# jesusbriales/dvo_slam

Measured on AMD Instinct MI355X. Metric: frame-pairs/s (640x480, 4-level GN align), higher is better.
Workload: dtype f32

## Files before the change

dvo_slam_amd/capi.py:

```python
from __future__ import annotations

import ctypes as C
import dataclasses
import os

import numpy as np

from . import _build

MAX_LEVELS = 8
TERMINATION = {0: "IterationsExceeded", 1: "IncrementTooSmall", 2: "LogLikelihoodDecreased", 3: "TooFewConstraints",
               -1: "Unset"}

EXPORTS = [
    "dvo_amd_abi_version", "dvo_amd_build_id", "dvo_amd_status_string", "dvo_amd_last_error", "dvo_amd_device_count",
    "dvo_amd_default_config", "dvo_amd_context_create", "dvo_amd_context_destroy", "dvo_amd_configure",
    "dvo_amd_get_config", "dvo_amd_pyramid_create", "dvo_amd_pyramid_create_from_device", "dvo_amd_pyramid_retain",
    "dvo_amd_pyramid_release", "dvo_amd_pyramid_levels", "dvo_amd_pyramid_timestamp", "dvo_amd_pyramid_level_info",
    "dvo_amd_pyramid_download_plane", "dvo_amd_pyramid_select", "dvo_amd_match", "dvo_amd_match_batch",
    "dvo_amd_residuals", "dvo_amd_error_image", "dvo_amd_kernel_timing", "dvo_amd_se3_exp", "dvo_amd_se3_log",
    "dvo_amd_solve6", "dvo_amd_bench_residual_pass", "dvo_amd_match_many",
    "dvo_amd_debug_finalize_stamps", "dvo_amd_comm_unique_id", "dvo_amd_comm_create", "dvo_amd_comm_destroy",
    "dvo_amd_match_sharded", "dvo_amd_match_banded", "dvo_amd_context_device", "dvo_amd_debug_combine_bands", "dvo_amd_debug_wire_layout", "dvo_amd_debug_take_wire", "dvo_amd_pyramid_create_raw",
    "dvo_amd_default_validator_stages", "dvo_amd_proposals_for_candidates", "dvo_amd_validate_proposals",
    "dvo_amd_track_frame", "dvo_amd_png_info", "dvo_amd_png_read_bgr8", "dvo_amd_png_read_gray16",
    "dvo_amd_format_trajectory_line", "dvo_amd_debug_tick_log", "dvo_amd_debug_iteration", "dvo_amd_match_selection", "dvo_amd_bench_residual_pass_pairs",
    "dvo_amd_exchange_create", "dvo_amd_exchange_attach", "dvo_amd_exchange_destroy",
    "dvo_amd_match_submit", "dvo_amd_match_wait", "dvo_amd_match_poll", "dvo_amd_debug_next_seq",
    "dvo_amd_set_reciprocal_mode", "dvo_amd_get_reciprocal_mode", "dvo_amd_debug_rcp", "dvo_amd_debug_block_trace",
    "dvo_amd_debug_ll_overflow", "dvo_amd_debug_marker", "dvo_amd_debug_rcp_form", "dvo_amd_debug_weights", "dvo_amd_debug_hw_queue",
    "dvo_amd_debug_level_geometry", "dvo_amd_point_cloud", "dvo_amd_map_cloud", "dvo_amd_voxel_downsample", "dvo_amd_write_pcd",
    "dvo_amd_debug_map_timing", "dvo_amd_default_graph_options", "dvo_amd_optimize_graph", "dvo_amd_graph_marginals", "dvo_amd_debug_graph_timing",
    "dvo_amd_debug_graph_system", "dvo_amd_debug_graph_system_sparse", "dvo_amd_debug_graph_symbolic",
    "dvo_amd_debug_graph_sparse_timing", "dvo_amd_optimize_graphs_batch", "dvo_amd_debug_graph_batch_records",
    "dvo_amd_debug_tick_layout",
    "dvo_amd_map_create", "dvo_amd_map_destroy", "dvo_amd_map_insert", "dvo_amd_map_set_poses", "dvo_amd_map_remove",
    "dvo_amd_map_stats", "dvo_amd_map_extract", "dvo_amd_map_render", "dvo_amd_map_render_pyramid", "dvo_amd_debug_keyframe_map_timing", "dvo_amd_debug_map_merge",
    "dvo_amd_default_covisibility_options", "dvo_amd_covisibility", "dvo_amd_find_constraint_candidates",
    "dvo_amd_debug_covisibility_ms",
    "dvo_amd_remap_create", "dvo_amd_remap_create_undistort", "dvo_amd_remap_retain", "dvo_amd_remap_release", "dvo_amd_remap_info",
    "dvo_amd_remap_download", "dvo_amd_pyramid_create_raw_remapped", "dvo_amd_debug_ingest_timing",
    "dvo_amd_default_registration", "dvo_amd_pyramid_create_raw_registered",
    "dvo_amd_pyramid_create_raw_batch", "dvo_amd_debug_batch_build_stats",
    "dvo_amd_mask_create", "dvo_amd_mask_create_levels", "dvo_amd_mask_retain", "dvo_amd_mask_release", "dvo_amd_mask_info",
    "dvo_amd_mask_download", "dvo_amd_pyramid_select_masked", "dvo_amd_match_masked", "dvo_amd_match_many_masked",
    "dvo_amd_default_budget_options", "dvo_amd_mask_create_budget",
    "dvo_amd_default_mask_warp_options", "dvo_amd_mask_combine", "dvo_amd_mask_morph", "dvo_amd_mask_warp", "dvo_amd_mask_warp_many",
    "dvo_amd_debug_mask_ops_timing",
    "dvo_amd_default_residual_mask_options", "dvo_amd_mask_from_residuals", "dvo_amd_mask_from_residuals_many",
    "dvo_amd_default_fuse_options", "dvo_amd_pyramid_fuse_depth", "dvo_amd_pyramid_fuse_depth_many", "dvo_amd_debug_fuse_timing",
    "dvo_amd_default_place_options", "dvo_amd_default_place_query_options", "dvo_amd_place_index_create", "dvo_amd_place_index_destroy",
    "dvo_amd_place_index_add", "dvo_amd_place_index_info", "dvo_amd_place_index_download", "dvo_amd_place_scores", "dvo_amd_place_query",
    "dvo_amd_place_query_frames", "dvo_amd_debug_place_timing",
    "dvo_amd_debug_residuals_masked", "dvo_amd_debug_iteration_masked", "dvo_amd_debug_weights_masked",
    "dvo_amd_default_normal_options", "dvo_amd_pyramid_normals", "dvo_amd_mask_from_normals", "dvo_amd_point_cloud_normals",
    "dvo_amd_write_pcd_normals", "dvo_amd_debug_normals_timing",
    "dvo_amd_default_depth_filter_options", "dvo_amd_pyramid_filter_depth", "dvo_amd_pyramid_filter_depth_many",
    "dvo_amd_debug_depth_filter_timing",
    "dvo_amd_default_component_options", "dvo_amd_mask_filter_components", "dvo_amd_mask_filter_components_many",
    "dvo_amd_mask_components", "dvo_amd_debug_components_timing",
    "dvo_amd_default_pose_score_options", "dvo_amd_score_poses", "dvo_amd_score_poses_many", "dvo_amd_rank_poses", "dvo_amd_pose_grid",
    "dvo_amd_default_exposure_options", "dvo_amd_estimate_exposure", "dvo_amd_estimate_exposure_many",
    "dvo_amd_pyramid_adjust_intensity", "dvo_amd_pyramid_adjust_intensity_many", "dvo_amd_debug_exposure_timing",
    "dvo_amd_default_warp_options", "dvo_amd_warp_inverse", "dvo_amd_warp_inverse_many", "dvo_amd_pyramid_warp_inverse",
    "dvo_amd_pyramid_warp_inverse_many", "dvo_amd_warp_forward", "dvo_amd_warp_forward_many", "dvo_amd_pyramid_warp_forward",
    "dvo_amd_pyramid_warp_forward_many", "dvo_amd_debug_warp_timing",
    "dvo_amd_default_volume_options", "dvo_amd_default_volume_raycast_options", "dvo_amd_volume_create", "dvo_amd_volume_destroy",
    "dvo_amd_volume_clear", "dvo_amd_volume_options_get", "dvo_amd_volume_integrate", "dvo_amd_volume_insert",
    "dvo_amd_volume_set_poses", "dvo_amd_volume_remove", "dvo_amd_volume_stats", "dvo_amd_volume_download", "dvo_amd_volume_raycast",
    "dvo_amd_volume_raycast_pyramid", "dvo_amd_volume_extract", "dvo_amd_debug_volume_timing",
    "dvo_amd_volume_mesh", "dvo_amd_volume_upload", "dvo_amd_write_ply",
]


class CConfig(C.Structure):
    _fields_ = [("first_level", C.c_int), ("last_level", C.c_int), ("max_iterations_per_level", C.c_int),
                ("precision", C.c_double), ("mu", C.c_double), ("use_initial_estimate", C.c_int),
                ("intensity_derivative_threshold", C.c_float), ("depth_derivative_threshold", C.c_float),
                ("segment_geometry", C.c_int), ("reserved", C.c_int)]


GEOMETRY_THROUGHPUT, GEOMETRY_LATENCY = 0, 1


class CIterationStats(C.Structure):
    _fields_ = [("id", C.c_int), ("valid_constraints", C.c_int), ("tdist_loglik", C.c_double),
                ("tdist_mean", C.c_double * 2), ("tdist_precision", C.c_double * 4), ("prior_loglik", C.c_double),
                ("increment", C.c_double * 6), ("information", C.c_double * 36), ("has_increment", C.c_int),
                ("reserved", C.c_int), ("estimate", C.c_double * 16), ("initial", C.c_double * 16)]


class CLevelStats(C.Structure):
    _fields_ = [("id", C.c_int), ("max_valid_pixels", C.c_int), ("valid_pixels", C.c_int), ("termination", C.c_int),
                ("n_iterations", C.c_int), ("first_iteration", C.c_int)]


class CResult(C.Structure):
    _fields_ = [("transformation", C.c_double * 16), ("information", C.c_double * 36), ("loglik", C.c_double),
                ("is_nan", C.c_int), ("n_levels", C.c_int), ("levels", CLevelStats * MAX_LEVELS),
                ("n_iterations", C.c_int), ("iterations_capacity", C.c_int),
                ("iterations", C.POINTER(CIterationStats)), ("n_ticks", C.c_int), ("n_residual_passes", C.c_int),
                ("alg_bytes", C.c_double), ("alg_bytes_discarded", C.c_double)]


class CFrameCriteria(C.Structure):
    _fields_ = [("odometry_is_nan", C.c_int), ("keyframe_is_nan", C.c_int), ("odometry_translation_norm", C.c_double),
                ("keyframe_translation_norm", C.c_double), ("keyframe_constraint_ratio", C.c_double),
                ("odometry_neg_loglik", C.c_double), ("keyframe_neg_loglik", C.c_double),
                ("odometry_condition_number", C.c_double), ("keyframe_condition_number", C.c_double)]


class CIterationProbe(C.Structure):
    _fields_ = [("valid_constraints", C.c_int), ("reserved", C.c_int), ("scale_sums", C.c_double * 3),
                ("scale", C.c_float * 4), ("precision", C.c_float * 4), ("moments", C.c_double * 87),
                ("information", C.c_double * 36), ("rhs", C.c_double * 6), ("loglik_sum", C.c_double),
                ("loglik", C.c_float), ("reserved_f", C.c_float)]


class CQ7Probe(C.Structure):
# ... 323 lines not shown
    L.dvo_amd_voxel_downsample.argtypes = [vp, C.c_longlong, vp, C.c_float, vp, C.c_longlong, C.POINTER(CCloudStats)]
    L.dvo_amd_write_pcd.argtypes = [C.c_char_p, vp, C.c_longlong, C.c_int, C.c_int]
    L.dvo_amd_debug_map_timing.argtypes = [vp, dp, dp, C.POINTER(C.c_longlong)]
    L.dvo_amd_map_create.argtypes = [vp, C.c_float, C.POINTER(vp)]
    L.dvo_amd_map_destroy.argtypes = [vp]
    L.dvo_amd_map_destroy.restype = None
    L.dvo_amd_map_insert.argtypes = [vp, C.c_int, vp, dp, vp, C.c_int]
    L.dvo_amd_map_set_poses.argtypes = [vp, C.c_int, C.POINTER(C.c_int), dp]
    L.dvo_amd_map_remove.argtypes = [vp, C.c_int, C.POINTER(C.c_int)]
    L.dvo_amd_map_stats.argtypes = [vp, C.POINTER(CCloudStats), C.POINTER(C.c_int)]
    L.dvo_amd_map_extract.argtypes = [vp, C.POINTER(C.c_float), vp, C.c_longlong, C.POINTER(C.c_longlong)]
    L.dvo_amd_map_render.argtypes = [vp, dp, C.POINTER(CView), vp, vp, vp, vp, C.POINTER(CRenderStats)]
    L.dvo_amd_map_render_pyramid.argtypes = [vp, dp, C.POINTER(CView), C.c_int, C.c_double, C.POINTER(vp), C.POINTER(CRenderStats)]
    L.dvo_amd_debug_keyframe_map_timing.argtypes = [vp, dp, dp, C.POINTER(C.c_longlong), C.POINTER(C.c_longlong),
                                                    C.POINTER(C.c_int)]
    L.dvo_amd_debug_map_merge.argtypes = [vp, C.c_longlong, vp, vp, C.c_longlong, vp, vp, vp, vp, C.POINTER(C.c_longlong)]
    L.dvo_amd_default_covisibility_options.argtypes = [C.POINTER(CCovisibilityOptions)]
    L.dvo_amd_default_covisibility_options.restype = None
    L.dvo_amd_covisibility.argtypes = [vp, C.c_int, C.POINTER(CKeyframe), C.POINTER(CCovisibilityOptions), C.c_int,
                                       C.POINTER(C.c_int), C.POINTER(C.c_int), vp]
    L.dvo_amd_find_constraint_candidates.argtypes = [vp, C.c_int, C.POINTER(CKeyframe), C.c_int, C.c_float, C.c_double,
                                                     C.POINTER(CCovisibilityOptions), C.POINTER(C.c_int), dp, C.c_int,
                                                     C.POINTER(C.c_int)]
    L.dvo_amd_debug_covisibility_ms.argtypes = [vp, dp]
    L.dvo_amd_remap_create.argtypes = [C.c_int, C.c_int, C.c_int, fp, fp, C.c_int, C.c_int, C.c_int, C.POINTER(vp)]
    L.dvo_amd_remap_create_undistort.argtypes = [C.c_int, C.c_int, C.c_int, fp, C.c_int, C.c_int, fp, fp, C.POINTER(vp)]
    L.dvo_amd_remap_retain.argtypes = [vp]
    L.dvo_amd_remap_retain.restype = None
    L.dvo_amd_remap_release.argtypes = [vp]
    L.dvo_amd_remap_release.restype = None
    L.dvo_amd_remap_info.argtypes = [vp, ip, ip, ip, ip, ip]
    L.dvo_amd_remap_download.argtypes = [vp, fp, fp]
    L.dvo_amd_pyramid_create_raw_remapped.argtypes = [C.c_int, vp, C.c_int, C.c_int, vp, C.c_int, C.c_float, C.c_int, vp,
                                                      C.c_float, C.c_float, C.c_float, C.c_float, C.c_int, C.c_double,
                                                      C.POINTER(vp)]
    L.dvo_amd_debug_ingest_timing.argtypes = [C.c_int, C.c_int, dp]
    L.dvo_amd_default_registration.argtypes = [C.POINTER(CRegistration)]
    L.dvo_amd_default_registration.restype = None
    L.dvo_amd_pyramid_create_raw_registered.argtypes = [C.c_int, vp, C.c_int, C.c_int, vp, C.c_int, C.c_float, C.c_int,
                                                        C.POINTER(CRegistration), vp, C.c_int, C.c_int, C.c_float, C.c_float,
                                                        C.c_float, C.c_float, C.c_int, C.c_double, C.POINTER(vp),
                                                        C.POINTER(CRegistrationStats)]
    L.dvo_amd_pyramid_create_raw_batch.argtypes = [C.c_int, C.POINTER(CRawBatch), C.POINTER(vp)]
    L.dvo_amd_debug_batch_build_stats.argtypes = [C.c_int, ip, ip, ip]
    L.dvo_amd_mask_create.argtypes = [C.c_int, C.c_int, C.c_int, C.c_int, vp, C.c_int, C.c_int, C.c_int, C.POINTER(vp)]
    L.dvo_amd_mask_create_levels.argtypes = [C.c_int, C.c_int, C.c_int, C.c_int, C.POINTER(vp), ip, C.c_int, C.POINTER(vp)]
    L.dvo_amd_mask_retain.argtypes = [vp]
    L.dvo_amd_mask_retain.restype = None
    L.dvo_amd_mask_release.argtypes = [vp]
    L.dvo_amd_mask_release.restype = None
    L.dvo_amd_mask_info.argtypes = [vp, ip, ip, ip, C.POINTER(C.c_longlong)]
    L.dvo_amd_mask_download.argtypes = [vp, C.c_int, C.POINTER(C.c_ubyte)]
    L.dvo_amd_pyramid_select_masked.argtypes = [vp, C.c_int, C.c_float, C.c_float, vp, C.POINTER(C.c_int), C.POINTER(C.c_ubyte)]
    L.dvo_amd_match_masked.argtypes = [vp, vp, vp, C.c_float, C.c_float, vp, dp, C.POINTER(CResult)]
    L.dvo_amd_match_many_masked.argtypes = [vp, C.c_int, C.POINTER(vp), C.POINTER(vp), C.POINTER(vp), dp, C.POINTER(CResult), C.c_int]
    L.dvo_amd_default_budget_options.argtypes = [C.POINTER(BudgetOptions)]
    L.dvo_amd_default_budget_options.restype = None
    L.dvo_amd_mask_create_budget.argtypes = [vp, C.POINTER(BudgetOptions), C.POINTER(vp)]
    L.dvo_amd_default_mask_warp_options.argtypes = [C.POINTER(MaskWarpOptions)]
    L.dvo_amd_default_mask_warp_options.restype = None
    L.dvo_amd_mask_combine.argtypes = [vp, vp, C.c_int, C.POINTER(vp)]
    L.dvo_amd_mask_morph.argtypes = [vp, C.c_int, ip, C.POINTER(vp)]
    L.dvo_amd_mask_warp.argtypes = [vp, vp, vp, dp, C.POINTER(MaskWarpOptions), C.POINTER(vp), C.POINTER(C.c_longlong)]
    L.dvo_amd_mask_warp_many.argtypes = [C.c_int, C.POINTER(vp), C.POINTER(vp), C.POINTER(vp), dp, C.POINTER(MaskWarpOptions),
                                         C.POINTER(vp), C.POINTER(C.c_longlong)]
    L.dvo_amd_debug_mask_ops_timing.argtypes = [C.c_int, C.c_int, dp]
    L.dvo_amd_default_residual_mask_options.argtypes = [C.POINTER(ResidualMaskOptions)]
    L.dvo_amd_default_residual_mask_options.restype = None
    L.dvo_amd_mask_from_residuals.argtypes = [vp, vp, vp, dp, C.POINTER(ResidualMaskOptions), C.POINTER(vp), C.POINTER(C.c_longlong),
                                              C.POINTER(C.POINTER(C.c_float))]
    L.dvo_amd_mask_from_residuals_many.argtypes = [vp, C.c_int, C.POINTER(vp), C.POINTER(vp), dp, C.POINTER(ResidualMaskOptions),
                                                   C.POINTER(vp), C.POINTER(C.c_longlong)]
    L.dvo_amd_default_pose_score_options.argtypes = [C.POINTER(PoseScoreOptions)]
    L.dvo_amd_default_pose_score_options.restype = None
    L.dvo_amd_score_poses.argtypes = [vp, vp, vp, C.c_int, dp, C.POINTER(PoseScoreOptions), vp]
    L.dvo_amd_score_poses_many.argtypes = [vp, C.c_int, C.POINTER(vp), C.POINTER(vp), ip, dp, C.POINTER(PoseScoreOptions), vp]
    L.dvo_amd_rank_poses.argtypes = [vp, C.c_int, C.c_int, ip, ip]
    L.dvo_amd_pose_grid.argtypes = [C.POINTER(PoseGridOptions), dp, dp, C.c_int, ip]
    L.dvo_amd_default_exposure_options.argtypes = [C.POINTER(ExposureOptions)]
    L.dvo_amd_default_exposure_options.restype = None
    L.dvo_amd_estimate_exposure.argtypes = [vp, vp, vp, dp, vp, C.POINTER(ExposureOptions), C.POINTER(ExposureEstimate)]
    L.dvo_amd_estimate_exposure_many.argtypes = [vp, C.c_int, C.POINTER(vp), C.POINTER(vp), dp, C.POINTER(vp),
                                                 C.POINTER(ExposureOptions), C.POINTER(ExposureEstimate)]
    L.dvo_amd_pyramid_adjust_intensity.argtypes = [vp, C.c_double, C.c_double, C.POINTER(vp)]
    L.dvo_amd_pyramid_adjust_intensity_many.argtypes = [C.c_int, C.POINTER(vp), dp, dp, C.POINTER(vp)]
    L.dvo_amd_debug_exposure_timing.argtypes = [C.c_int, C.c_int, dp]
    L.dvo_amd_default_warp_options.argtypes = [C.POINTER(WarpOptions)]
    L.dvo_amd_default_warp_options.restype = None
    ll, wo, cv = C.POINTER(C.c_longlong), C.POINTER(WarpOptions), C.POINTER(CView)
    L.dvo_amd_warp_inverse.argtypes = [vp, vp, dp, C.c_int, wo, fp, fp, ll]
    L.dvo_amd_warp_inverse_many.argtypes = [C.c_int, C.POINTER(vp), C.POINTER(vp), dp, C.c_int, wo, C.POINTER(vp), C.POINTER(vp), ll]
    L.dvo_amd_pyramid_warp_inverse.argtypes = [vp, vp, dp, wo, C.POINTER(vp), ll]
    L.dvo_amd_pyramid_warp_inverse_many.argtypes = [C.c_int, C.POINTER(vp), C.POINTER(vp), dp, wo, C.POINTER(vp), ll]
    L.dvo_amd_warp_forward.argtypes = [vp, dp, cv, C.c_int, wo, fp, fp, ip, ll]
    L.dvo_amd_warp_forward_many.argtypes = [C.c_int, C.POINTER(vp), dp, cv, C.c_int, wo, C.POINTER(vp), C.POINTER(vp), C.POINTER(vp), ll]
    L.dvo_amd_pyramid_warp_forward.argtypes = [vp, dp, cv, wo, C.POINTER(vp), ll]
    L.dvo_amd_pyramid_warp_forward_many.argtypes = [C.c_int, C.POINTER(vp), dp, cv, wo, C.POINTER(vp), ll]
    L.dvo_amd_debug_warp_timing.argtypes = [C.c_int, C.c_int, ip, ip, dp]
    vo, ro = C.POINTER(VolumeOptions), C.POINTER(VolumeRaycastOptions)
    L.dvo_amd_default_volume_options.argtypes = [vo]
    L.dvo_amd_default_volume_options.restype = None
    L.dvo_amd_default_volume_raycast_options.argtypes = [ro]
    L.dvo_amd_default_volume_raycast_options.restype = None
    L.dvo_amd_volume_create.argtypes = [C.c_int, vo, C.POINTER(vp)]
    L.dvo_amd_volume_destroy.argtypes = [vp]
    L.dvo_amd_volume_destroy.restype = None
# ... 1017 lines not shown
        b.timestamps = None if timestamps is None else (C.c_double * n)(*[float(t) for t in timestamps])
        b.channels, b.image_stride_bytes, b.depth_stride = channels, image_stride_bytes or w * channels, depth_stride or w
        b.depth_scale, b.on_device, b.width, b.height = depth_scale, int(on_device), w, h
        b.fx, b.fy, b.ox, b.oy = [float(k) for k in K]
        b.levels, b.build_selection = levels, int(selection is not None)
        if selection is not None:
            b.intensity_threshold, b.depth_threshold = float(selection[0]), float(selection[1])
        out = (C.c_void_p * n)()
        _check(lib().dvo_amd_pyramid_create_raw_batch(device, C.byref(b), out), "dvo_amd_pyramid_create_raw_batch")
        del keep
        pyramids = []
        for f in range(n):
            self = cls.__new__(cls)
            self._h, self.device, self.registration_stats = C.c_void_p(out[f]), device, None
            pyramids.append(self)
        return pyramids

    def __del__(self):
        h = getattr(self, "_h", None)
        if h:
            lib().dvo_amd_pyramid_release(h)
            self._h = None

    def levels(self) -> int:
        return lib().dvo_amd_pyramid_levels(self._h)

    def timestamp(self) -> float:
        return lib().dvo_amd_pyramid_timestamp(self._h)

    def level_info(self, level: int):
        w, h = C.c_int(), C.c_int()
        k = np.zeros(4, np.float32)
        _check(lib().dvo_amd_pyramid_level_info(self._h, level, C.byref(w), C.byref(h), _fp(k)), "level_info")
        return w.value, h.value, k

    def plane(self, level: int, plane: int) -> np.ndarray:
        w, h, _ = self.level_info(level)
        out = np.empty((h, w), np.float32)
        _check(lib().dvo_amd_pyramid_download_plane(self._h, level, plane, _fp(out)), "download_plane")
        return out

    def select(self, level: int, ti: float = 0.0, td: float = 0.0, mask: "SelectionMask | None" = None):
        w, h, _ = self.level_info(level)
        out = np.empty((h, w), np.uint8)
        cnt = C.c_int()
        if mask is not None:
            _check(lib().dvo_amd_pyramid_select_masked(self._h, level, ti, td, mask._h, C.byref(cnt),
                                                       out.ctypes.data_as(C.POINTER(C.c_ubyte))), "pyramid_select_masked")
            return cnt.value, out
        _check(lib().dvo_amd_pyramid_select(self._h, level, ti, td, C.byref(cnt),
                                            out.ctypes.data_as(C.POINTER(C.c_ubyte))), "pyramid_select")
        return cnt.value, out


    def fuse_depth(self, frames, transformations, options=None, counts: bool = False, observations: bool = False):
        got = RgbdImagePyramid.fuse_depth_many([self], [frames], [transformations], options, counts=counts, observations=observations)
        return tuple(part[0] for part in got) if counts or observations else got[0]

    @staticmethod
    def fuse_depth_many(keyframes, frames_per_keyframe, transformations_per_keyframe, options=None, counts: bool = False,
                        observations: bool = False):
        nk = len(keyframes)
        if not (len(frames_per_keyframe) == len(transformations_per_keyframe) == nk):
            raise ValueError("one list of frames and one list of transformations per keyframe")
        if any(len(f) != len(t) for f, t in zip(frames_per_keyframe, transformations_per_keyframe)):
            raise ValueError("one transformation per frame")
        opt = options if isinstance(options, FuseOptions) else fuse_options(**(options or {}))
        vp = C.c_void_p
        offsets = np.concatenate([[0], np.cumsum([len(f) for f in frames_per_keyframe])]).astype(np.int32)
        total = int(offsets[-1])
        flat = [p for f in frames_per_keyframe for p in f]
        T = np.ascontiguousarray(np.stack([_pose_cm(t) for ts in transformations_per_keyframe for t in ts]) if total
                                 else np.zeros((1, 4, 4)), dtype=np.float64)
        frame_cnt = np.zeros(max(1, total), FUSE_FRAME_DTYPE)
        key_cnt = np.zeros(max(1, nk), FUSE_KEYFRAME_DTYPE)
        planes = []
        for kf in keyframes:
            w, h, _ = kf.level_info(0)
            planes.append(np.zeros((h, w), np.uint8))
        out = (vp * max(1, nk))()
        obs = (vp * max(1, nk))(*[p.ctypes.data for p in planes]) if observations else None
        ll = C.POINTER(C.c_longlong)
        _check(lib().dvo_amd_pyramid_fuse_depth_many(nk, (vp * max(1, nk))(*[p._h for p in keyframes]),
                                                     offsets.ctypes.data_as(C.POINTER(C.c_int)),
                                                     (vp * max(1, total))(*[p._h for p in flat]), T.ctypes.data_as(C.POINTER(C.c_double)),
                                                     C.byref(opt), out, frame_cnt.ctypes.data_as(ll) if counts else None,
                                                     key_cnt.ctypes.data_as(ll) if counts else None, obs),
               "dvo_amd_pyramid_fuse_depth_many")
        made = []
        for j in range(nk):
            p = RgbdImagePyramid.__new__(RgbdImagePyramid)
            p._h, p.device, p.registration_stats = vp(out[j]), keyframes[j].device, None
            made.append(p)
        result = (made,)
        if counts:
            result += ([frame_cnt[offsets[j]:offsets[j + 1]].copy() for j in range(nk)], key_cnt[:nk].copy())
        if observations:
            result += (planes,)
        return result if len(result) > 1 else made


    def warp_inverse(self, fixed: "RgbdImagePyramid", T, level=None, options=None):
        got = warp_inverse_many([fixed], [self], [T], level, options)
        return tuple(part[0] for part in got)

    def warp_forward(self, T, view=None, level=None, options=None):
# ... 1028 lines not shown
```

dvo_slam_amd/csrc/dvo_internal.h:

```cpp
#pragma once
#include <hip/hip_runtime.h>
#include <rccl/rccl.h>

#include <atomic>
#include <cmath>
#include <cstddef>
#include <deque>
#include <memory>
#include <mutex>
#include <string>
#include <vector>

#include "../../include/dvo_amd.h"
#include "../../include/dvo_amd_debug.h"
#include "dvo_launch_rules.h"
#include "dvo_types.h"
#include "se3.h"

namespace dvo_amd {
namespace host {

extern thread_local std::string g_last_error;
int fail_hip(const char *what, hipError_t e);

// ... 4 lines not shown
  } while (0)

inline size_t align_up(size_t v, size_t a) { return (v + a - 1) / a * a; }

inline int invalid(const char *entry, const std::string &why) {
  g_last_error = std::string(entry) + ": " + why;
  return DVO_AMD_ERR_INVALID_ARGUMENT;
}

template <typename T>
inline bool finite_all(const T *v, int n) {
  for (int i = 0; i < n; ++i)
    if (!std::isfinite(v[i])) return false;
  return true;
}

inline int have_device(int *count = nullptr) {
  int ndev = 0;
  if (hipGetDeviceCount(&ndev) != hipSuccess || ndev <= 0) return DVO_AMD_ERR_NO_DEVICE;
  if (count) *count = ndev;
  return DVO_AMD_OK;
}

constexpr int kSpecLevelsMaxPairs = 8;
constexpr size_t kTickLogFields = 8;
constexpr int kMaxTickStreams = 8;

constexpr int kMaxDevices = 16;
constexpr int kMaxBands = 16;

}
}

using namespace dvo_amd;


struct CompactLevel {
  float *z, *i, *ix, *iy, *tx, *ty;
  int *pix;
};
constexpr size_t kCompactBytesPerPoint = 7 * sizeof(float);
struct Selection {
  float ti, td;
  unsigned long long mask_serial = 0;
  float *zsel[DVO_AMD_MAX_LEVELS];
  CompactLevel pts[DVO_AMD_MAX_LEVELS];
  int count[DVO_AMD_MAX_LEVELS];
  int n_pts[DVO_AMD_MAX_LEVELS];
  int last[DVO_AMD_MAX_LEVELS];
  RefLevelDesc *ref_desc;
  void *desc_entry = nullptr;
  void *extra_slab;
  size_t extra_bytes;
};

struct LevelData {
  int w, h, n, n_pad;
  float fx, fy, ox, oy;
  float *i_plane, *z_plane;
  float4 *c_a;
  float2 *c_b;
  float *r_i, *r_ix, *r_iy;
  float *tx, *ty;
  float *zsel0;
  char *pts0;
};

struct dvo_amd_pyramid {
  std::atomic<int> refs{1};
  int device = 0;
  int n_levels = 0;
  double timestamp = 0.0;
  LevelData lv[DVO_AMD_MAX_LEVELS];
  void *slab = nullptr;
  size_t slab_bytes = 0;
  int *counters = nullptr;
  int2 *sel_partials = nullptr;
  int *sel_prefix = nullptr;
  void *desc_entry = nullptr;
  CurLevelDesc *cur_desc = nullptr;
  RefLevelDesc *ref_desc0 = nullptr;
  std::mutex mu;
  std::vector<std::unique_ptr<Selection>> selections;
};

struct dvo_amd_remap {
  std::atomic<int> refs{1};
  int device = 0;
  int w = 0, h = 0;
  int sw = 0, sh = 0;
  int n_inside = 0;
  void *mem = nullptr;
  float *map_x = nullptr, *map_y = nullptr;
  int *counter = nullptr;
};

struct dvo_amd_mask {
  std::atomic<int> refs{1};
  int device = 0;
  int w = 0, h = 0, levels = 0;
  unsigned long long serial = 0;
  void *mem = nullptr;
  unsigned char *plane[DVO_AMD_MAX_LEVELS] = {};
  int *counters = nullptr;
  long long kept[DVO_AMD_MAX_LEVELS] = {};
};
// ... 66 lines not shown
  int device = 0;
  dvo_amd_config cfg;
  hipStream_t stream = nullptr;
  std::vector<hipStream_t> extra_streams;
  hipEvent_t desc_ready = nullptr;
  std::vector<JobSlot> slots;
  int slot_n_pad = 0;
  FinWire *out_wire = nullptr;
  std::vector<FinOut> out_store;
  FinOut *out_host = nullptr;
  int out_capacity = 0;
  SlotDesc *slot_desc = nullptr;
  Runner *runner = nullptr;
  int items_per_launch = kMaxItemsPerLaunch;
  int ll_merge = 4;
  int spec_levels = -1;
  bool host_prof = false;
  double prof_submit_ns = 0.0, prof_wait_ns = 0.0, prof_process_ns = 0.0;
  long long prof_ticks = 0, prof_job_ticks = 0;
  void *rccl_lib = nullptr;
  ncclComm_t comm = nullptr;
  int comm_ranks = 0, comm_rank = 0;
  FinOut *gather_dev = nullptr, *gather_host = nullptr;
  FinWire *xbuf = nullptr;
  FinWire *xpeers[kMaxExchangeRanks] = {};
  bool xpeer_opened[kMaxExchangeRanks] = {};
  int x_ranks = 0, x_rank = 0;
  FinWire *x_host = nullptr;
  FinOut x_store[kMaxExchangeRanks];
  unsigned *x_host_seq = nullptr;
  unsigned x_seq = 0;
  bool x_broken = false;
  ExchangeArgs *x_args_dev = nullptr;
  ncclResult_t (*p_allgather)(const void *, void *, size_t, ncclDataType_t, ncclComm_t, hipStream_t) = nullptr;
  ncclResult_t (*p_comm_destroy)(ncclComm_t) = nullptr;
  unsigned tick_seq = 0;
  RcpTable rcp = {nullptr, 0, 0, nullptr};
  unsigned *rcp_table_dev = nullptr;
  unsigned *rcp_nibbles_dev = nullptr;
  int rcp_unit = 0;
  std::string rcp_form_note;
  int q7_off256 = 0;
  float *dbg_w_dev = nullptr;
  size_t dbg_w_capacity = 0;
  unsigned *ovf_host = nullptr, *ovf_dev = nullptr;
  long long ovf_checks = 0, ovf_hits = 0;
  long long level_steps_at[5] = {18, 70, 1000, 1000, 1LL << 40};
  long long level_steps_at_latency[5] = {250, 4000, 38400, 999999, 1LL << 40};
  int fine_steps = 0;
  int fault_slot_alloc = -1;
  bool fin_stamps = false;
  bool sort_items = true;
  int share_placement = 1;
  bool fin_priority = true;
  bool small_args = true;
  bool poll = true;
  bool timing = false;
  double timing_ms = 0.0;
  long long timing_launches = 0;
  std::vector<double> tick_log;
  std::vector<double> tick_log_pending;
  std::vector<std::pair<hipEvent_t, hipEvent_t>> events;
  size_t events_used = 0;
  host::MapWorkspace *map_ws = nullptr;
  host::GraphWorkspace *graph_ws = nullptr;
  host::GraphBatchWorkspace *graph_batch_ws = nullptr;
  host::CovisWorkspace *covis_ws = nullptr;
};

namespace dvo_amd {
namespace host {

struct IterCtx {
  int k = 0;
  int buf = 0;
  int steps = 4;
  int n_blocks = 0;
  SE3 inc;
  SE3 initial_before, estimate_before;
  SE3 initial_after, estimate_after;
  double x_before[6];
  int n = 0;
  float cov[4], P[4];
  double A[36], b[6], x_new[6], prior = 0.0;
  int cut_rank = 0;
  int band_valid[kMaxBands];
  bool cont = false;
  int stats_index = -1;
};

struct Job {
  dvo_amd_pyramid *ref = nullptr, *cur = nullptr;
  const Selection *sel = nullptr;
  dvo_amd_result *result = nullptr;
  JobSlot *slot = nullptr;
  const dvo_amd_config *cfg = nullptr;
  int level = 0, iteration = 0;
  SE3 inc, initial, estimate;
  double x[6];
  double error = DBL_MAX, last_error = DBL_MAX;
  float precision[4] = {0, 0, 0, 0};
  bool done = false;
  int status = DVO_AMD_OK;
  bool have_a = false, have_b = false;
  bool sub_ll = false, sub_res = false;
  IterCtx a, b;
  IterCtx spec_b;
  bool have_spec = false;
  double sub_px = 0.0;
  int buf_flip = 0;
  int next_flip = 0;
  dvo_amd_iteration_stats recent[2];
  int recent_count = 0;
  int level_first_iteration = 0;
  double alg_px = 0.0;
  double discarded_px = 0.0;
};

struct GroupTick {
  size_t lo = 0, hi = 0;
  size_t stream_first = 0;
  int id = 0;
  unsigned seq = 0;
  bool in_flight = false;
};

struct OvfBand {
  int seg_first, n_segs, rank_offset;
  int rank_end = -1;
};
}
}

using namespace dvo_amd::host;

struct Pending {
  dvo_amd_pyramid *ref = nullptr, *cur = nullptr;
  dvo_amd_result *result = nullptr;
  unsigned long long batch = 0;
  bool has_init = false;
  double T_init[16];
  float ti = 0.0f, td = 0.0f;
  dvo_amd_mask *mask = nullptr;
};
struct Batch {
  unsigned long long id = 0;
  int remaining = 0;
};
struct Runner {
  std::vector<Job> jobs;
  std::vector<unsigned long long> batch_of_slot;
  std::vector<GroupTick> groups;
  std::deque<Pending> pending;
  std::deque<Batch> batches;
  unsigned long long next_batch = 1;
  size_t next_group = 0;
  int in_flight = 0;
  bool timing = false;
  int resident = 0;
  struct Failure {
    unsigned long long batch;
    int status;
  };
  std::vector<Failure> failures;
  int unreported_failure = DVO_AMD_OK;
};

namespace dvo_amd {
namespace host {

int device_prep_stream(int device, hipStream_t *s);
int slab_alloc(int device, size_t bytes, void **out);
int desc_alloc(int device, void **out);
void desc_free(int device, void *p);
void slab_free(int device, size_t bytes, void *p);
int pyramid_selection(dvo_amd_pyramid *p, float ti, float td, const dvo_amd_mask *mask, const Selection **out);
inline int pyramid_selection(dvo_amd_pyramid *p, float ti, float td, const Selection **out) {
  return pyramid_selection(p, ti, td, nullptr, out);
}
int mask_fits(const char *entry, const dvo_amd_pyramid *p, const dvo_amd_mask *mask);
std::mutex &device_mutex(int device);
int pyramid_build(int device, const PyramidSpec &spec, const Level0Source &src, dvo_amd_pyramid **out);
int ingest_timing(int device, int enable, double *last_ms);
int pyramid_build_batch(int device, const dvo_amd_raw_batch &b, dvo_amd_pyramid **out);
int batch_build_stats(int device, int *kernel_launches, int *copies, int *synchronisations);

int ingest_level0(int device, const PyramidSpec &spec, const Level0Source &src, const LevelData &L0, unsigned long long *ctrl,
                  hipStream_t st);
int check_levels(const char *entry, int w, int h, int levels, const char *of = "");

int check_mask_size(const char *entry, int width, int height, int levels);
int mask_alloc(const char *entry, int device, int width, int height, int levels, dvo_amd_mask **out, hipStream_t *st);
int mask_finish(dvo_amd_mask *m, hipError_t e, hipStream_t st, dvo_amd_mask **out);

int launch_remap_ingest(const dvo_amd_remap *r, const unsigned char *d_img, int channels, int img_stride, unsigned char *grey,
                        int grey_stride, const unsigned short *d_z, int z_stride, float z_scale, float *i_plane, float *z_plane,
                        hipStream_t st);

int launch_register_depth(const Registration &R, const unsigned short *d_z, int z_stride, float z_scale, float *z_plane,
                          const PyramidSpec &view, unsigned long long *ctrl, hipStream_t st);

dvo_amd_iteration_stats *stats_push(Job &j);
void stats_publish(Job &j);
void begin_iteration(Job &j, IterCtx &it, int k);
void finish_job(Job &j);
void end_level(Job &j);
void start_level(Job &j);
void speculate_next_level(const Job &j, IterCtx &b_out);
void make_kt(const LevelData &C, const SE3 &estimate, float kt[12]);
int blocks_for(int n, int steps);
int level_blocks(const Selection *sel, int level, int steps);
void scale_and_precision(const FinOut &o, int n, float cov[4], float P[4]);
void system_from_moments(const FinOut &o, const float P[4], double mu, const double xi_initial[6], double A[36], double b[6]);
float loglik_from_sum(int n, const float P[4], double ll_sum, bool overflowed = false);
void process_residual(Job &j, IterCtx &it, const FinOut &o);
void process_loglik(Job &j, const FinOut *outs, bool ll_overflowed = false);
void release_slots(dvo_amd_context *ctx);
int ensure_slots_impl(dvo_amd_context *ctx, int n_jobs, int n_pad);
int ensure_slots(dvo_amd_context *ctx, int n_jobs, int n_pad);
int level_steps(const dvo_amd_context *ctx, const LevelData &lv);
int level_ll_merge(const dvo_amd_context *ctx, int res_steps);
int timing_begin(dvo_amd_context *ctx, size_t *slot);
int tick_stream(dvo_amd_context *ctx, size_t index, hipStream_t *out);
int probe_hw_queue(dvo_amd_context *ctx, int *pipe_queue);
int timing_collect(dvo_amd_context *ctx);
int take_wire(const FinWire *w, FinOut *dst_record, unsigned seq, int from_piece);
int take_record(dvo_amd_context *ctx, size_t slot, unsigned seq, int from_piece);
int take_record_synced(dvo_amd_context *ctx, size_t slot, unsigned seq);
int wait_tick(dvo_amd_context *ctx, const std::vector<Job> &jobs, size_t lo, size_t hi, unsigned seq);
int submit_tick(dvo_amd_context *ctx, std::vector<Job> &jobs, GroupTick &grp);
int ll_overflowed(dvo_amd_context *ctx, const float2 *res, const int *seg_prefix, int n_blocks, int steps, int cut_rank,
                  const float P[4], const OvfBand *bands, int n_bands, bool *overflowed);
// ... 30 lines not shown
```

dvo_slam_amd/csrc/dvo_kernels.hip:

```cpp
#include <algorithm>
#include <cstddef>
#include <cstdlib>
#include <cstring>
#include <functional>
#include <mutex>
#include <vector>

#include "dvo_launch_rules.h"
#include "dvo_types.h"

namespace dvo_amd {


#define DVO_HWREG_MODE_FP32_ROUND (1 | (0 << 6) | ((2 - 1) << 11))
#define DVO_OPAQUE(x) asm volatile("" : "+v"(x))
#ifndef DVO_KT_SGPR
#define DVO_KT_SGPR 1
#endif

__device__ __forceinline__ void round_toward_zero() { __builtin_amdgcn_s_setreg(DVO_HWREG_MODE_FP32_ROUND, 3); }
__device__ __forceinline__ void round_to_nearest() { __builtin_amdgcn_s_setreg(DVO_HWREG_MODE_FP32_ROUND, 0); }

__device__ __forceinline__ float mul_legacy(float a, float b) {
  float r;
// ... 36 lines not shown
  if (__builtin_expect(az < 1.1754944e-38f || az > 8.5070592e+37f, 0)) return 1.0f / z;
  const float r = __builtin_amdgcn_rcpf(az);
  const float e = __builtin_fmaf(-az, r, 1.0f);
  const unsigned lo = f2u(__builtin_fmaf(e, r, r));
  const unsigned up = lo + 1u;
  const bool up_fits = __builtin_fmaf(-az, u2f(up), 1.0f) >= 0.0f;
  return __builtin_copysignf(u2f(up_fits ? up : lo), z);
}

__device__ __forceinline__ float rcp_host_table(float z, const RcpTable &rcp) {
  const unsigned u = f2u(z), au = u & 0x7fffffffu, e = au >> 23, m = au & 0x7fffffu;
  const unsigned t = ((const __attribute__((address_space(1))) unsigned *)rcp.table)[m >> rcp.shift];
  const int re = (int)(t >> 23) - ((int)e - 127);
  unsigned r = re >= 1 ? (((unsigned)re << 23) | (t & 0x7fffffu)) : 0u;
  r = e == 0u ? 0x7f800000u : r;
  r = e == 255u ? (m ? (au | 0x00400000u) : 0u) : r;
  return u2f(r | (u & 0x80000000u));
}

__device__ __forceinline__ unsigned rcp_midpoint_bits(unsigned cell, int shift) {
  return f2u(__builtin_amdgcn_rcpf(u2f(0x3f800000u | (cell << shift) | (1u << (shift - 1)))));
}
template <bool NAN_ANY>
__device__ __forceinline__ float rcp_host_nibbles(float z, const unsigned *lds_nib, int shift, int unit) {
  const unsigned u = f2u(z), au = u & 0x7fffffffu, e = au >> 23, m = au & 0x7fffffu;
  const unsigned cell = m >> shift;
  const unsigned word = lds_nib[cell >> 3];
  const int corr = (int)(((word >> ((cell & 7u) * 4u)) & 15u) ^ 8u) - 8;
  const unsigned t = (rcp_midpoint_bits(cell, shift) & ~((1u << unit) - 1u)) + (unsigned)(corr << unit);
  unsigned r = t - ((e - 127u) << 23);
  if (__builtin_expect(__builtin_amdgcn_ballot_w64(e - 1u >= 252u && !(NAN_ANY && au > 0x7f800000u)) != 0ull, 0)) {
    const int re = (int)(t >> 23) - ((int)e - 127);
    r = re >= 1 ? (((unsigned)re << 23) | (t & 0x7fffffu)) : 0u;
    r = e == 0u ? 0x7f800000u : r;
    r = e == 255u ? (m ? (au | 0x00400000u) : 0u) : r;
  }
  return u2f(r | (u & 0x80000000u));
}

#define DVO_GLOBAL __attribute__((address_space(1)))
typedef float v4f __attribute__((ext_vector_type(4)));
typedef float v2f __attribute__((ext_vector_type(2)));
typedef float v4f_a8 __attribute__((ext_vector_type(4), aligned(8)));
typedef const DVO_GLOBAL float *gcf;
template <class T, int IMM = 0>
__device__ __forceinline__ T ld_off(const DVO_GLOBAL void *base, unsigned byte_off) {
  return *reinterpret_cast<const DVO_GLOBAL T *>(reinterpret_cast<const DVO_GLOBAL char *>(base) + byte_off + IMM);
}
typedef const DVO_GLOBAL v4f *gcf4;


struct LevelPairDesc {
  const float *r_zsel, *r_i, *r_ix, *r_iy, *tx, *ty;
  const float4 *c_a;
  const float2 *c_b;
  float2 *res[2];
  float *records;
  double *ll_partials;
  float *ll_qmax;
  int *seg_prefix[2];
  int w, h;
  float wc[6], wr[4], ub_x, ub_y;
  RcpTable rcp;
  const unsigned *rcp_lds;
  float *dbg_w;
};

#ifdef DVO_TRACE_BLOCKS
struct BlockTrace {
  unsigned long long t0, t_first, t_end;
  unsigned info;
  unsigned hw;
};
constexpr unsigned kTraceCapacity = 1u << 22;
__device__ BlockTrace g_trace[kTraceCapacity];
__device__ unsigned g_trace_n;
__device__ __forceinline__ unsigned long long trace_clock() { return __builtin_amdgcn_s_memrealtime(); }
__shared__ unsigned long long trace_first;
__shared__ unsigned long long trace_tail;
#endif


struct Proj {
  float u, v, sz;
  int base;
  bool inb;
};
struct Gathered {
  v4f a00, a10, a01, a11;
  v4f_a8 b0, b1;
};

template <int RCP>
__device__ __forceinline__ Proj project_pixel_rtz(const float *kt, const LevelPairDesc &d, float x, float y, float z) {
  const float sx = (kt[0] * x + kt[1] * y) + (kt[2] * z + kt[3]);
  const float sy = (kt[4] * x + kt[5] * y) + (kt[6] * z + kt[7]);
  Proj p;
  p.sz = (kt[8] * x + kt[9] * y) + (kt[10] * z + kt[11]);
  const float rz = RCP == 2   ? rcp_host_nibbles<true>(p.sz, d.rcp_lds, d.rcp.shift, d.rcp.unit)
                   : RCP == 1 ? rcp_host_table(p.sz, d.rcp)
                              : rcp_toward_zero(p.sz);
  p.u = sx * rz, p.v = sy * rz;
  p.inb = (bool)((int)(p.u >= 0.0f) & (int)(p.u <= d.ub_x) & (int)(p.v >= 0.0f) & (int)(p.v <= d.ub_y));
  const int iu = (int)p.u, iv = (int)p.v;
  p.base = p.inb ? __mul24(iv, d.w) + iu : 0;
  return p;
}

__device__ __forceinline__ Gathered gather_pixel(const LevelPairDesc &d, int base) {
  const DVO_GLOBAL void *ca = (const DVO_GLOBAL void *)d.c_a, *cb = (const DVO_GLOBAL void *)d.c_b;
  const unsigned oa0 = (unsigned)base * 16u, oa1 = oa0 + (unsigned)d.w * 16u;
  const unsigned ob0 = (unsigned)base * 8u, ob1 = ob0 + (unsigned)d.w * 8u;
  Gathered g;
  g.a00 = ld_off<v4f>(ca, oa0), g.a10 = ld_off<v4f, 16>(ca, oa0);
  g.a01 = ld_off<v4f>(ca, oa1), g.a11 = ld_off<v4f, 16>(ca, oa1);
  g.b0 = ld_off<v4f_a8>(cb, ob0);
  g.b1 = ld_off<v4f_a8>(cb, ob1);
  return g;
}

template <class T>
__device__ __forceinline__ void st_once(DVO_GLOBAL T *p, const T v) {
  __builtin_nontemporal_store(v, p);
}
template <class T>
__device__ __forceinline__ T ld_once(const DVO_GLOBAL T *p) {
  return __builtin_nontemporal_load(p);
}

template <bool ZERO_E>
__device__ __forceinline__ void finish_pixel_rtz(const LevelPairDesc &d, const Proj &p, const Gathered &g, float z, float ri,
                                                 float rix, float riy, float &r0, float &r1, float &e2, float &e3, float &e4,
                                                 float &e5, bool &valid) {
  const float w1u = __builtin_amdgcn_fractf(p.u), w1v = __builtin_amdgcn_fractf(p.v);
  const float w0u = 1.0f - w1u, w0v = 1.0f - w1v;
#define DVO_BLEND(c00, c10, c01, c11) ((w0v * (w0u * (c00) + w1u * (c10))) + (w1v * (w0u * (c01) + w1u * (c11))))
  const float ci = DVO_BLEND(g.a00.x, g.a10.x, g.a01.x, g.a11.x);
  const float cz = DVO_BLEND(g.a00.y, g.a10.y, g.a01.y, g.a11.y);
  const float cix = DVO_BLEND(g.a00.z, g.a10.z, g.a01.z, g.a11.z);
  const float ciy = DVO_BLEND(g.a00.w, g.a10.w, g.a01.w, g.a11.w);
  const float czx = DVO_BLEND(g.b0.x, g.b0.z, g.b1.x, g.b1.z);
  const float czy = DVO_BLEND(g.b0.y, g.b0.w, g.b1.y, g.b1.w);
#undef DVO_BLEND
  const bool has_nan = __builtin_isunordered(ci, cz) || __builtin_isunordered(cix, ciy) || __builtin_isunordered(czx, czy);
  const float t0 = d.wc[0] * ci + d.wr[0] * ri;
  const float t1 = d.wc[1] * cz + d.wr[1] * p.sz;
  float s = z - 0.4f;
  s = 0.0012f + (0.0019f * s) * s;
  valid = p.inb && !has_nan && (t1 > -20.0f * s);
  r0 = valid ? t0 : 0.0f;
  r1 = valid ? t1 : 0.0f;
  e2 = d.wc[2] * cix + d.wr[2] * rix;
  e3 = d.wc[3] * ciy + d.wr[3] * riy;
  e4 = d.wc[4] * czx;
  e5 = d.wc[5] * czy;
  if (ZERO_E) e2 = valid ? e2 : 0.0f, e3 = valid ? e3 : 0.0f, e4 = valid ? e4 : 0.0f, e5 = valid ? e5 : 0.0f;
}

typedef float v4acc __attribute__((ext_vector_type(4)));
#ifndef DVO_GRAM_BLOCKS
#define DVO_GRAM_BLOCKS 1
#endif
constexpr int kGramPairs = 9;
__host__ __device__ constexpr int gram_pair(int ci, int cj) { return ci == 0 ? cj : ci == 1 ? 3 + cj : 5 + cj; }

#define DVO_WAVE_LDS_SYNC()                                 \
  do {                                                      \
    __builtin_amdgcn_fence(__ATOMIC_ACQ_REL, "wavefront");  \
    __builtin_amdgcn_wave_barrier();                        \
  } while (0)

#ifndef DVO_ABLATE
#define DVO_ABLATE 0
#endif
#define DVO_KEEP(x) asm volatile("" ::"v"(x))

template <int ACC, int RCP>
__device__ void residual_pass(const TickItem &it, const LevelPairDesc &d_in, const int lb) {
  LevelPairDesc d = d_in;
  __shared__ unsigned rcp_lds[RCP == 2 ? kRcpNibbleWordsMax : 1];
  if (RCP == 2) {
    const int words = (1 << (23 - d.rcp.shift)) >> 3;
    for (int i = threadIdx.x; i < words; i += kBlockThreads) rcp_lds[i] = ((const DVO_GLOBAL unsigned *)d.rcp.nibbles)[i];
    __syncthreads();
    d.rcp_lds = rcp_lds;
  }
  constexpr int kBufs = 2;
  const int lane = threadIdx.x & (kWave - 1);
  const int wave = threadIdx.x >> 6;
  const int wave_s = __builtin_amdgcn_readfirstlane(wave);
  const int seg = lb * kWavesPerBlock + wave;
  const int steps = item_res_steps(it);
  unsigned idx = (unsigned)(seg * (kStepPx * steps) + lane);

  float acc[ACC == 0 ? kNumAcc : 1];
#pragma unroll
  for (int i = 0; i < (ACC == 0 ? kNumAcc : 1); ++i) acc[i] = 0.0f;
  v4acc gram_a = {0.0f, 0.0f, 0.0f, 0.0f}, gram_b = {0.0f, 0.0f, 0.0f, 0.0f};
  v4acc gram_p[kGramPairs];
#pragma unroll
  for (int k = 0; k < kGramPairs; ++k) gram_p[k] = v4acc{0.0f, 0.0f, 0.0f, 0.0f};
  __shared__ __attribute__((aligned(16))) float stage[ACC >= 1 ? kWavesPerBlock * kBufs * kWave * 16 : 4];
  float S0[3] = {0.0f, 0.0f, 0.0f}, S1[3] = {0.0f, 0.0f, 0.0f};
  float first_w = 0.0f;
  int run_count = 0;
  __shared__ __attribute__((aligned(8))) v2f pair_slots[kWavesPerBlock][kWave + 2];
  v2f *const slots = pair_slots[wave];
  if (lane == 0) slots[0] = v2f{0.0f, 0.0f};

  float kt[12];
#pragma unroll
  for (int i = 0; i < 12; ++i) {
    kt[i] = it.kt[i];
    if (DVO_KT_SGPR)
      asm volatile("" : "+s"(kt[i]));
    else
      DVO_OPAQUE(kt[i]);
  }
  const bool unit_w = (it.flags & kItemUnitWeights) != 0;
  const float P0 = it.P[0], P1 = it.P[1], P2 = it.P[2], P3 = it.P[3];
  const DVO_GLOBAL void *const p_z = (const DVO_GLOBAL void *)d.r_zsel, *const p_i = (const DVO_GLOBAL void *)d.r_i,
                         *const p_ix = (const DVO_GLOBAL void *)d.r_ix, *const p_iy = (const DVO_GLOBAL void *)d.r_iy,
                         *const p_tx = (const DVO_GLOBAL void *)d.tx, *const p_ty = (const DVO_GLOBAL void *)d.ty;
  DVO_GLOBAL char *const p_res = (DVO_GLOBAL char *)((it.flags & kItemResBuf) ? d.res[1] : d.res[0]);

  float n_z, n_i, n_ix, n_iy, n_tx, n_ty;
  auto load_first = [&](const bool opaque) __attribute__((always_inline)) {
    unsigned at = idx;
    if (opaque) DVO_OPAQUE(at);
    n_z = ld_off<float>(p_z, 4u * at), n_i = ld_off<float>(p_i, 4u * at), n_ix = ld_off<float>(p_ix, 4u * at),
    n_iy = ld_off<float>(p_iy, 4u * at);
    n_tx = ld_off<float>(p_tx, 4u * at), n_ty = ld_off<float>(p_ty, 4u * at);
  };

  const int g_comp = lane & 15, g_sub = lane >> 4, g_cb = (g_comp >> 2) ^ (g_sub >> 1);
  const float *const g_even = stage + (wave * kBufs * kWave + g_sub) * 16 + ((g_cb << 2) | (g_comp & 3));
  const float *const g_odd = stage + (wave * kBufs * kWave + g_sub) * 16 + (((g_cb ^ 2) << 2) | (g_comp & 3));
  const int b_swz = (lane >> 3) & 3;
  const float *const b_base = stage + (wave * kBufs * kWave + (lane >> 2)) * 16 + (lane & 3);
  const float *const b_c0 = b_base + 4 * (0 ^ b_swz), *const b_c1 = b_base + 4 * (1 ^ b_swz), *const b_c2 = b_base + 4 * (2 ^ b_swz),
                     *const b_c3 = b_base + 4 * (3 ^ b_swz);
  auto gram_from_stage = [&](const int q) __attribute__((always_inline)) {
    if (DVO_GRAM_BLOCKS) {
#pragma unroll
      for (int g = 0; g < 4; ++g) {
        const int off = (q & (kBufs - 1)) * kWave * 16 + g * 16 * 16;
        const float x0 = b_c0[off], x1 = b_c1[off], x2 = b_c2[off], x3 = b_c3[off];
        gram_p[0] = __builtin_amdgcn_mfma_f32_4x4x1f32(x0, x0, gram_p[0], 0, 0, 0);
        gram_p[1] = __builtin_amdgcn_mfma_f32_4x4x1f32(x0, x1, gram_p[1], 0, 0, 0);
        gram_p[2] = __builtin_amdgcn_mfma_f32_4x4x1f32(x0, x2, gram_p[2], 0, 0, 0);
        gram_p[3] = __builtin_amdgcn_mfma_f32_4x4x1f32(x0, x3, gram_p[3], 0, 0, 0);
        gram_p[4] = __builtin_amdgcn_mfma_f32_4x4x1f32(x1, x1, gram_p[4], 0, 0, 0);
        gram_p[5] = __builtin_amdgcn_mfma_f32_4x4x1f32(x1, x2, gram_p[5], 0, 0, 0);
        gram_p[6] = __builtin_amdgcn_mfma_f32_4x4x1f32(x1, x3, gram_p[6], 0, 0, 0);
        gram_p[7] = __builtin_amdgcn_mfma_f32_4x4x1f32(x2, x2, gram_p[7], 0, 0, 0);
        gram_p[8] = __builtin_amdgcn_mfma_f32_4x4x1f32(x2, x3, gram_p[8], 0, 0, 0);
      }
      return;
    }
#pragma unroll
    for (int m = 0; m < 16; m += 2) {
      const float va = g_even[(q & (kBufs - 1)) * kWave * 16 + 64 * m];
      const float vb = g_odd[(q & (kBufs - 1)) * kWave * 16 + 64 * (m + 1)];
      gram_a = __builtin_amdgcn_mfma_f32_16x16x4f32(va, va, gram_a, 0, 0, 0);
      gram_b = __builtin_amdgcn_mfma_f32_16x16x4f32(vb, vb, gram_b, 0, 0, 0);
    }
  };

  auto do_step = [&](const int step, const int q, const bool prefetch) __attribute__((always_inline)) {
    const unsigned cur_idx = idx;
    float z = n_z, ri = n_i, rix = n_ix, riy = n_iy;
    float x = n_tx * z, y = n_ty * z;
    idx += kWave;
    auto prefetch_next = [&]() __attribute__((always_inline)) {
      n_z = ld_off<float>(p_z, 4u * idx), n_i = ld_off<float>(p_i, 4u * idx), n_ix = ld_off<float>(p_ix, 4u * idx),
      n_iy = ld_off<float>(p_iy, 4u * idx);
      n_tx = ld_off<float>(p_tx, 4u * idx), n_ty = ld_off<float>(p_ty, 4u * idx);
    };

    DVO_OPAQUE(x); DVO_OPAQUE(y); DVO_OPAQUE(z); DVO_OPAQUE(ri); DVO_OPAQUE(rix); DVO_OPAQUE(riy);
    round_toward_zero();
    DVO_OPAQUE(x); DVO_OPAQUE(y); DVO_OPAQUE(z); DVO_OPAQUE(ri); DVO_OPAQUE(rix); DVO_OPAQUE(riy);
    float r0, r1, e2, e3, e4, e5;
    bool ok;
    {
      const Proj p = project_pixel_rtz<RCP>(kt, d, x, y, z);
      Gathered g;
      if (DVO_ABLATE & 2) {
        const v4f c = {p.u, 1.5f, p.v, 0.25f};
        g.a00 = c, g.a10 = c, g.a01 = c, g.a11 = c, g.b0 = c, g.b1 = c;
        DVO_KEEP(p.base);
      } else {
        g = gather_pixel(d, p.base);
        if (ACC >= 1 && !(DVO_ABLATE & 1) && step > 0) __builtin_amdgcn_sched_barrier(0);
      }

      if (ACC >= 1 && !(DVO_ABLATE & 1) && step > 0) {
        gram_from_stage(q ^ 1);
        __builtin_amdgcn_sched_barrier(0);
      }
      if (prefetch) prefetch_next();
      finish_pixel_rtz<ACC == 0>(d, p, g, z, ri, rix, riy, r0, r1, e2, e3, e4, e5, ok);
    }
    DVO_OPAQUE(r0); DVO_OPAQUE(r1); DVO_OPAQUE(e2); DVO_OPAQUE(e3); DVO_OPAQUE(e4); DVO_OPAQUE(e5);
    DVO_OPAQUE(x); DVO_OPAQUE(y); DVO_OPAQUE(z);
    round_to_nearest();
    DVO_OPAQUE(r0); DVO_OPAQUE(r1); DVO_OPAQUE(e2); DVO_OPAQUE(e3); DVO_OPAQUE(e4); DVO_OPAQUE(e5);
    DVO_OPAQUE(x); DVO_OPAQUE(y); DVO_OPAQUE(z);

    {
      const float qnan = u2f(0x7fc00000u);
      v2f sv;
      sv.x = ok ? r0 : qnan, sv.y = ok ? r1 : qnan;
      if (DVO_ABLATE & 8) {
        DVO_KEEP(sv.x);
        DVO_KEEP(sv.y);
      } else {
        st_once(reinterpret_cast<DVO_GLOBAL v2f *>(p_res + 8u * cur_idx), sv);
      }
    }

    float wgt = 1.0f;
    if (!unit_w) {
      const float t0 = RCP ? r0 * P0 + r1 * P1 : __builtin_fmaf(r0, P0, r1 * P1);
      const float t1 = RCP ? r0 * P2 + r1 * P3 : __builtin_fmaf(r0, P2, r1 * P3);
      const float dd = RCP ? t0 * r0 + t1 * r1 : __builtin_fmaf(t0, r0, t1 * r1);
      wgt = 7.0f * (RCP == 2   ? rcp_host_nibbles<true>(5.0f + dd, d.rcp_lds, d.rcp.shift, d.rcp.unit)
                    : RCP == 1 ? rcp_host_table(5.0f + dd, d.rcp)
                               : __builtin_amdgcn_rcpf(5.0f + dd));
    }
    wgt = ok ? wgt : 0.0f;
    if (RCP && d.dbg_w) ((DVO_GLOBAL float *)d.dbg_w)[cur_idx] = ok ? wgt : u2f(0x7fc00000u);

    x = ok ? x : 0.0f, y = ok ? y : 0.0f, z = ok ? z : 1.0f;
    const float iz = __builtin_amdgcn_rcpf(z);
    const float iz2 = iz * iz;
    const float j02 = -x * iz2, j12 = -y * iz2;
    const float j03 = j02 * y, j13 = __builtin_fmaf(j12, y, -1.0f);
    const float j04 = __builtin_fmaf(-j02, x, 1.0f), j14 = -j03;
    const float j05 = -y * iz, j15 = x * iz;
    const float sw = ACC == 0 ? 1.0f : __builtin_amdgcn_sqrtf(wgt);
    const float g2 = ACC == 0 ? e2 : mul_legacy(sw, e2), g3 = ACC == 0 ? e3 : mul_legacy(sw, e3);
    const float g4 = ACC == 0 ? e4 : mul_legacy(sw, e4), g5 = ACC == 0 ? e5 : mul_legacy(sw, e5);
    const float swx = sw * x, swy = sw * y;
    float Ja[6], Jb[6];
    Ja[0] = g2 * iz;
    Ja[1] = g3 * iz;
    Ja[2] = __builtin_fmaf(g2, j02, g3 * j12);
    Ja[3] = __builtin_fmaf(g2, j03, g3 * j13);
    Ja[4] = __builtin_fmaf(g2, j04, g3 * j14);
    Ja[5] = __builtin_fmaf(g2, j05, g3 * j15);
    Jb[0] = g4 * iz;
    Jb[1] = g5 * iz;
    Jb[2] = __builtin_fmaf(g4, j02, __builtin_fmaf(g5, j12, -sw));
    Jb[3] = __builtin_fmaf(g4, j03, __builtin_fmaf(g5, j13, -swy));
    Jb[4] = __builtin_fmaf(g4, j04, __builtin_fmaf(g5, j14, swx));
    Jb[5] = __builtin_fmaf(g4, j05, g5 * j15);
    if (ACC == 0) {
      float wa[6], wb[6];
#pragma unroll
      for (int i = 0; i < 6; ++i) wa[i] = wgt * Ja[i], wb[i] = wgt * Jb[i];
      int t = 0;
#pragma unroll
      for (int i = 0; i < 6; ++i) {
#pragma unroll
        for (int j = i; j < 6; ++j, ++t) {
          acc[kAccAA + t] = __builtin_fmaf(wa[i], Ja[j], acc[kAccAA + t]);
          acc[kAccAB + t] = __builtin_fmaf(wa[i], Jb[j], __builtin_fmaf(wb[i], Ja[j], acc[kAccAB + t]));
          acc[kAccBB + t] = __builtin_fmaf(wb[i], Jb[j], acc[kAccBB + t]);
        }
        acc[kAccAR0 + i] = __builtin_fmaf(wa[i], r0, acc[kAccAR0 + i]);
        acc[kAccAR1 + i] = __builtin_fmaf(wa[i], r1, acc[kAccAR1 + i]);
        acc[kAccBR0 + i] = __builtin_fmaf(wb[i], r0, acc[kAccBR0 + i]);
        acc[kAccBR1 + i] = __builtin_fmaf(wb[i], r1, acc[kAccBR1 + i]);
      }
    } else if (DVO_ABLATE & 1) {
#pragma unroll
      for (int i = 0; i < 6; ++i) {
        DVO_KEEP(Ja[i]);
        DVO_KEEP(Jb[i]);
      }
      DVO_KEEP(wgt);
    } else {
      float *buf = stage + ((wave_s * kBufs + (q & (kBufs - 1))) * kWave) * 16;
      v4f *row = reinterpret_cast<v4f *>(buf + lane * 16);
      const int swz = (lane >> 1) & 3;
      v4f c0 = {Ja[0], Ja[1], Ja[2], Ja[3]};
      v4f c1 = {Ja[4], Ja[5], Jb[0], Jb[1]};
      v4f c2 = {Jb[2], Jb[3], Jb[4], Jb[5]};
      v4f c3 = {sw * r0, sw * r1, 0.0f, 0.0f};
      __builtin_amdgcn_fence(__ATOMIC_ACQ_REL, "wavefront");
      __builtin_amdgcn_wave_barrier();
      row[0 ^ swz] = c0;
      row[1 ^ swz] = c1;
      row[2 ^ swz] = c2;
      row[3 ^ swz] = c3;
      __builtin_amdgcn_fence(__ATOMIC_ACQ_REL, "wavefront");
      __builtin_amdgcn_wave_barrier();
    }

    if (DVO_ABLATE & 4) {
      S0[0] += wgt * r0;
      run_count += __popcll(__ballot(ok));
      return;
    }
    const unsigned long long bk = __builtin_amdgcn_ballot_w64(ok);
    const int pos = (int)__builtin_amdgcn_mbcnt_hi((unsigned)(bk >> 32), __builtin_amdgcn_mbcnt_lo((unsigned)bk, 0u));
    const int rank = run_count + pos;
    const int n_here = __popcll(bk);
    DVO_WAVE_LDS_SYNC();
    if (ok) slots[pos + 1] = v2f{r0, r1};
    DVO_WAVE_LDS_SYNC();
    const v2f prev = slots[pos];
    DVO_WAVE_LDS_SYNC();
    if (n_here) slots[0] = slots[n_here];
    {
      const bool odd = (rank & 1) != 0;
      const float a0 = odd ? prev.x : r0, a1 = odd ? prev.y : r1;
      const float b0 = odd ? r0 : prev.x, b1 = odd ? r1 : prev.y;
      S0[0] = __builtin_fmaf(wgt, a0 * a0, S0[0]);
      S0[1] = __builtin_fmaf(wgt, a0 * a1, S0[1]);
      S0[2] = __builtin_fmaf(wgt, a1 * a1, S0[2]);
      S1[0] = __builtin_fmaf(wgt, b0 * b0, S1[0]);
      S1[1] = __builtin_fmaf(wgt, b0 * b1, S1[1]);
      S1[2] = __builtin_fmaf(wgt, b1 * b1, S1[2]);
      first_w = (ok && rank == 0) ? wgt : first_w;
    }
    run_count += n_here;
  };
  if (!(DVO_ABLATE & 16)) {
    if (steps == 1) {
      load_first(true);
      do_step(0, 1, false);
#if defined(DVO_TRACE_BLOCKS) && !defined(DVO_TRACE_DESC)
      if (threadIdx.x == 0) trace_first = trace_clock();
#endif
    } else {
#ifdef DVO_TRACE_BLOCKS
      bool marked = false;
#endif
      load_first(false);
      for (int step = 0; step + 2 < steps; step += 2) {
        do_step(step, 0, true);
#if defined(DVO_TRACE_BLOCKS) && !defined(DVO_TRACE_DESC)
        if (!marked && threadIdx.x == 0) trace_first = trace_clock();
        marked = true;
#endif
        do_step(step + 1, 1, true);
      }
      do_step(steps - 2, 0, true);
#if defined(DVO_TRACE_BLOCKS) && !defined(DVO_TRACE_DESC)
      if (!marked && threadIdx.x == 0) trace_first = trace_clock();
#endif
      do_step(steps - 1, 1, false);
    }
  }

  if (DVO_ABLATE & 32) {
    float keep = S0[0] + S1[0] + first_w + gram_a[0] + gram_b[0] + (float)run_count;
    for (int k = 0; k < kGramPairs; ++k) keep += gram_p[k][0];
    DVO_KEEP(keep);
    return;
  }
  if (ACC >= 1 && !(DVO_ABLATE & 1) && steps > 0) gram_from_stage(1);

  __shared__ float sm[kWavesPerBlock][kRecStride];
  if (ACC == 0) {
#pragma unroll
    for (int i = 0; i < kNumAcc; ++i) {
      const float s = wave_sum_to_lane63(acc[i]);
      if (lane == 63) sm[wave][kRecAcc + i] = s;
    }
  } else {
    float *gsm = stage + wave_s * kBufs * kWave * 16;
    __builtin_amdgcn_fence(__ATOMIC_ACQ_REL, "wavefront");
    __builtin_amdgcn_wave_barrier();
    if (DVO_GRAM_BLOCKS) {
#pragma unroll
      for (int k = 0; k < kGramPairs; ++k) {
        v4acc t = gram_p[k];
#pragma unroll
        for (int r = 0; r < 4; ++r) {
          float v = t[r];
          v += dpp_read<0x124, 0xF>(v);
          v += dpp_read<0x128, 0xF>(v);
          t[r] = v;
        }
        if ((lane & 12) == 0) *reinterpret_cast<v4f *>(gsm + ((k * 4 + (lane >> 4)) * 4 + (lane & 3)) * 4) = v4f{t[0], t[1], t[2], t[3]};
      }
    } else {
#pragma unroll
      for (int r = 0; r < 4; ++r) gsm[((lane >> 4) * 4 + r) * 16 + (lane & 15)] = gram_a[r] + gram_b[r];
    }
  }
#pragma unroll
  for (int i = 0; i < 3; ++i) {
    const float s0 = (DVO_ABLATE & 64) ? S0[i] : wave_sum_to_lane63(S0[i]);
    const float s1 = (DVO_ABLATE & 64) ? S1[i] : wave_sum_to_lane63(S1[i]);
    if (lane == 63) sm[wave][kRecS0 + i] = s0, sm[wave][kRecS1 + i] = s1;
  }
  {
    const float fw = (DVO_ABLATE & 64) ? first_w : wave_sum_to_lane63(first_w);
    if (lane == 63) {
      const v2f last = slots[0];
      sm[wave][kRecFirstW] = fw;
      sm[wave][kRecCount] = u2f((unsigned)run_count);
      sm[wave][kRecLastR] = last.x;
      sm[wave][kRecLastR + 1] = last.y;
    }
  }
  const int tid = threadIdx.x;
  int e0 = 0, e1 = -1;
  if (ACC >= 1 && tid < kNumAcc) {
    if (tid < kAccAR0) {
      const int kind = tid / 21;
      int t = tid - kind * 21, i = 0;
      while (t >= 6 - i) t -= 6 - i, ++i;
      const int j = i + t;
      if (kind == 0) {
        e0 = i * 16 + j;
      } else if (kind == 1) {
        e0 = i * 16 + 6 + j, e1 = j * 16 + 6 + i;
      } else {
        e0 = (6 + i) * 16 + 6 + j;
      }
    } else {
      const int q = tid - kAccAR0, grp = q / 6, i = q - grp * 6;
      e0 = ((grp >> 1) * 6 + i) * 16 + 12 + (grp & 1);
    }
    if (DVO_GRAM_BLOCKS) {
      auto at = [](const int e) { return ((gram_pair((e >> 4) >> 2, (e & 15) >> 2) * 4) * 4 + (e & 3)) * 4 + ((e >> 4) & 3); };
      e0 = at(e0);
      if (e1 >= 0) e1 = at(e1);
    }
  }
  __syncthreads();

  DVO_GLOBAL float *rec = (DVO_GLOBAL float *)d.records + (size_t)lb * kRecStride;
  if ((DVO_ABLATE & 128) && tid < kNumAcc) {
    st_once(rec + kRecAcc + tid, stage[tid]);
  } else if ((DVO_ABLATE & 256) && tid == 128) {
    st_once(rec + kRecCount, sm[0][kRecCount]);
  } else if (tid < kNumAcc) {
    if (ACC == 0) {
      st_once(rec + kRecAcc + tid, (sm[0][kRecAcc + tid] + sm[1][kRecAcc + tid]) + (sm[2][kRecAcc + tid] + sm[3][kRecAcc + tid]));
    } else {
      constexpr int kW = kBufs * kWave * 16;
      float v;
      if (DVO_GRAM_BLOCKS) {
        auto rows = [&](const float *p) { return (p[0] + p[16]) + (p[32] + p[48]); };
        auto waves = [&](const int e) { return (rows(stage + e) + rows(stage + kW + e)) + (rows(stage + 2 * kW + e) + rows(stage + 3 * kW + e)); };
        v = waves(e0);
        if (e1 >= 0) v += waves(e1);
      } else {
        v = (stage[e0] + stage[kW + e0]) + (stage[2 * kW + e0] + stage[3 * kW + e0]);
        if (e1 >= 0) v += (stage[e1] + stage[kW + e1]) + (stage[2 * kW + e1] + stage[3 * kW + e1]);
      }
      st_once(rec + kRecAcc + tid, v);
    }
  } else if (tid == 128) {
    unsigned CB[kWavesPerBlock];
    float FW[kWavesPerBlock], L0[kWavesPerBlock], L1[kWavesPerBlock], A0[kWavesPerBlock][3], A1[kWavesPerBlock][3];
#pragma unroll
    for (int wv = 0; wv < kWavesPerBlock; ++wv) {
// ... 148 lines not shown
  if (rank_end >= 0) {
    const int closed = rank_end - rank_end % 50;
    stop = stop < closed ? stop : closed;
    px_end = (seg_first + n_segs) * seg_px;
  }
  if (first >= stop) return;
  int run = a, base = first;
  bool overflow = false;
  auto flush = [&](int n_groups) {
    __syncthreads();
    if (lane < n_groups) {
      double acc = 1.0;
      for (int i = 0; i < 50; ++i) acc *= terms[lane * 50 + i];
      overflow = overflow || !(acc <= 1.7976931348623157e308);
    }
    __syncthreads();
  };
  for (int i0 = s0 * seg_px; i0 < px_end && run < stop; i0 += kWave) {
    const float2 r = res[i0 + lane];
    const bool valid = r.x == r.x;
    const unsigned long long b = __ballot(valid);
    const int rank = run + __popcll(b & below);
    if (valid && rank >= first && rank < stop) {
      const float t0 = r.x * P0 + r.y * P1;
      const float t1 = r.x * P2 + r.y * P3;
      const float q = t0 * r.x + t1 * r.y;
      terms[rank - base] = 1.0 + 0.2 * (double)q;
    }
    run += __popcll(b);
    const int have = (run < stop ? run : stop) - base;
    if (have >= kOvfWindow) {
      flush(kOvfGroups);
      const double t = terms[kOvfWindow + lane];
      __syncthreads();
      if (lane < have - kOvfWindow) terms[lane] = t;
      __syncthreads();
      base += kOvfWindow;
    }
  }
  const int left = (run < stop ? run : stop) - base;
  if (left >= 50) flush(left / 50);
  const unsigned long long any = __ballot(overflow);
  if (lane == 0 && any) __hip_atomic_store(result_host, 1u, __ATOMIC_RELAXED, __HIP_MEMORY_SCOPE_SYSTEM);
}

#define DVO_CONST __attribute__((address_space(4)))
__device__ __forceinline__ LevelPairDesc load_desc(const TickItem &it) {
  const DVO_CONST RefLevelDesc *r = (const DVO_CONST RefLevelDesc *)it.ref;
  const DVO_CONST CurLevelDesc *c = (const DVO_CONST CurLevelDesc *)it.cur;
  const DVO_CONST SlotDesc *s = (const DVO_CONST SlotDesc *)it.slot;
  LevelPairDesc d;
  d.r_zsel = r->r_zsel, d.r_i = r->r_i, d.r_ix = r->r_ix, d.r_iy = r->r_iy;
  d.tx = r->tx, d.ty = r->ty;
  d.c_a = c->c_a, d.c_b = c->c_b;
  d.w = c->w, d.h = c->h;
#pragma unroll
  for (int i = 0; i < 6; ++i) d.wc[i] = c->wc[i];
#pragma unroll
  for (int i = 0; i < 4; ++i) d.wr[i] = c->wr[i];
  d.ub_x = c->ub_x, d.ub_y = c->ub_y;
  d.res[0] = s->res[0], d.res[1] = s->res[1];
  d.records = s->records, d.ll_partials = s->ll_partials, d.ll_qmax = s->ll_qmax;
  d.seg_prefix[0] = s->seg_prefix[0], d.seg_prefix[1] = s->seg_prefix[1];
  return d;
}

template <int ACC, int RCP>
__device__ __forceinline__ void tick_body(const TickItem &it, const RcpTable &rcp, const int bx) {
  const int rb = it.res_blocks;
  if (bx >= rb + it.ll_blocks) return;
#ifdef DVO_TRACE_BLOCKS
  const unsigned long long trace_t0 = trace_clock();
  unsigned trace_slot = 0;
  if (threadIdx.x == 0) trace_first = 0, trace_tail = 0, trace_slot = atomicAdd(&g_trace_n, 1u);
#endif
  LevelPairDesc d = load_desc(it);
#ifdef DVO_TRACE_DESC
  if (threadIdx.x == 0) {
    asm volatile("s_waitcnt lgkmcnt(0)" ::: "memory");
    DVO_KEEP(d.w);
    trace_first = trace_clock();
  }
#endif
  d.rcp = rcp;
  d.rcp_lds = nullptr;
  d.dbg_w = RCP ? ((const DVO_CONST SlotDesc *)it.slot)->dbg_w : nullptr;
  if (bx < rb)
    residual_pass<ACC, RCP>(it, d, it.res_first + xcd_contiguous_block(bx, rb));
  else
    loglik_pass(it, d, (int)it.ll_first + (bx - rb));
#ifdef DVO_TRACE_BLOCKS
  if (threadIdx.x == 0) {
    const unsigned long long trace_t1 = trace_clock();
    const unsigned slot = trace_slot;
    if (slot < kTraceCapacity) {
      unsigned hw, xcc;
      asm volatile("s_getreg_b32 %0, hwreg(HW_REG_HW_ID)" : "=s"(hw));
      asm volatile("s_getreg_b32 %0, hwreg(HW_REG_XCC_ID)" : "=s"(xcc));
      BlockTrace t;
      t.t0 = trace_t0, t.t_first = trace_first, t.t_end = trace_t1;
#ifdef DVO_TRACE_TAIL
      if (bx < rb) {
        const unsigned long long t_spin = trace_clock();
        unsigned long long tail = 0;
        while ((tail = __hip_atomic_load(&trace_tail, __ATOMIC_RELAXED, __HIP_MEMORY_SCOPE_WORKGROUP)) == 0 && trace_clock() - t_spin < 2000) {}
        t.t_first = tail;
      }
#endif
      t.info = (unsigned)(bx < rb ? (it.steps_log2 & 15) : (it.steps_log2 >> 4)) | (bx < rb ? 0u : 16u) | ((unsigned)(d.w / 8) << 8) |
               ((unsigned)(bx < rb ? rb : it.ll_blocks) << 16);
      t.hw = (hw & 0x0fffffffu) | (xcc << 28);
      g_trace[slot] = t;
    }
  }
#endif
}

template <class Args>
__host__ __device__ __forceinline__ int tick_place(const Args &args, int idx, int pos, const unsigned block, int &bx) {
  if constexpr (Args::kSets) {
    if (args.compact > 1) {
      const unsigned m = args.set_size[idx];
      if (m > 1) {
        const unsigned q = (unsigned)(((unsigned long long)(unsigned)pos * args.set_inv[idx]) >> 32);
        idx += pos - (int)(q * m);
        pos = (int)q;
      }
    }
  }
  const int rot = pos < (int)(args.items[idx].res_blocks >> 3) ? args.xcd_rot[idx] : args.tail_rot[idx];
  bx = (pos << 3) | (int)((block + (unsigned)rot) & 7u);
  return idx;
}

template <class Args>
__device__ __forceinline__ int tick_locate(const Args &args, int &bx, const unsigned block = blockIdx.x) {
  constexpr int kSlots = (int)(sizeof(args.group_first) / sizeof(args.group_first[0]));
  if (!args.compact) return tick_place(args, (int)blockIdx.y, (int)(block >> 3), block, bx);
  const int lane = threadIdx.x & (kWave - 1);
  const unsigned g = block >> 3;
  const unsigned first = lane <= args.n_items ? (unsigned)args.group_first[lane < kSlots ? lane : 0] : 0xFFFFFFFFu;
  const int idx = __builtin_amdgcn_readfirstlane(__popcll(__ballot(first <= g)) - 1);
// ... 29 lines not shown
  for (int o = kWave / 2; o; o >>= 1) v += __shfl_xor(v, o);
  const int n_tail = (it.flags & kItemUnitWeights) ? 0 : (v & 3);
  __shared__ double sh_delta[3][3 + kNumAcc];
  __shared__ int sh_idx[3];
  __shared__ float sh_r0[3], sh_r1[3];
  if (lane < 3) {
    sh_idx[lane] = 0, sh_r0[lane] = sh_r1[lane] = 0.0f;
    for (int i = 0; i < 3 + kNumAcc; ++i) sh_delta[lane][i] = 0.0;
  }
  __syncthreads();
  int found = 0;
  if (n_tail) {
    const DVO_GLOBAL v2f *const res = (const DVO_GLOBAL v2f *)((it.flags & kItemResBuf) ? d.res[1] : d.res[0]);
    for (int sg = nb * kWavesPerBlock - 1; sg >= 0 && found < n_tail; --sg) {
      const int c = __builtin_amdgcn_readfirstlane((int)f2u(recs[(size_t)(sg >> 2) * kRecStride + kRecWaveCnt + (sg & 3)]));
      if (c == 0) continue;
      for (int st = steps - 1; st >= 0 && found < n_tail; --st) {
        const int first = sg * seg_px + st * kStepPx;
        const v2f r = res[first + lane];
        unsigned long long m = __ballot(r.x == r.x);
        while (m && found < n_tail) {
          const int hi = 63 - __builtin_clzll(m);
          const float r0 = __shfl(r.x, hi), r1 = __shfl(r.y, hi);
          if (lane == 0) sh_idx[found] = first + hi, sh_r0[found] = r0, sh_r1[found] = r1;
          m &= ~(1ull << hi);
          ++found;
        }
      }
    }
    __syncthreads();
  }
  const bool mine = lane < n_tail && found == n_tail;
  float w_table = 0.0f, w_exact = 0.0f;
  bool equal = true;
  int my_idx = 0;
  if (n_tail && found == n_tail) {
    const int j = lane < n_tail ? lane : 0;
    const int k = n_tail - 1 - j;
    const unsigned idx = (unsigned)sh_idx[k];
    my_idx = (int)idx;
    float z = ((gcf)d.r_zsel)[idx], ri = ((gcf)d.r_i)[idx], rix = ((gcf)d.r_ix)[idx], riy = ((gcf)d.r_iy)[idx];
    float x = ((gcf)d.tx)[idx] * z, y = ((gcf)d.ty)[idx] * z;
    float kt[12];
#pragma unroll
    for (int i = 0; i < 12; ++i) kt[i] = it.kt[i];
    DVO_OPAQUE(x); DVO_OPAQUE(y); DVO_OPAQUE(z); DVO_OPAQUE(ri); DVO_OPAQUE(rix); DVO_OPAQUE(riy);
    round_toward_zero();
    DVO_OPAQUE(x); DVO_OPAQUE(y); DVO_OPAQUE(z); DVO_OPAQUE(ri); DVO_OPAQUE(rix); DVO_OPAQUE(riy);
    float r0, r1, e2, e3, e4, e5;
    bool ok;
    {
      const Proj p = project_pixel_rtz<1>(kt, d, x, y, z);
      const Gathered g = gather_pixel(d, p.base);
      finish_pixel_rtz<true>(d, p, g, z, ri, rix, riy, r0, r1, e2, e3, e4, e5, ok);
    }
    DVO_OPAQUE(r0); DVO_OPAQUE(r1); DVO_OPAQUE(e2); DVO_OPAQUE(e3); DVO_OPAQUE(e4); DVO_OPAQUE(e5);
    DVO_OPAQUE(x); DVO_OPAQUE(y); DVO_OPAQUE(z);
    round_to_nearest();
    DVO_OPAQUE(r0); DVO_OPAQUE(r1); DVO_OPAQUE(e2); DVO_OPAQUE(e3); DVO_OPAQUE(e4); DVO_OPAQUE(e5);
    DVO_OPAQUE(x); DVO_OPAQUE(y); DVO_OPAQUE(z);
    equal = ok && f2u(r0) == f2u(sh_r0[k]) && f2u(r1) == f2u(sh_r1[k]);
    const float t0 = r0 * it.P[0] + r1 * it.P[1];
    const float t1 = r0 * it.P[2] + r1 * it.P[3];
    const float dd = t0 * r0 + t1 * r1;
    w_table = 7.0f * rcp_host_table(5.0f + dd, d.rcp);
    w_exact = (float)((2.0 + 5.0f) / (5.0f + dd));
    const double dw = mine ? (double)w_exact - (double)w_table : 0.0;
    const float iz = __builtin_amdgcn_rcpf(z);
    const float iz2 = iz * iz;
    const float j02 = -x * iz2, j12 = -y * iz2;
    const float j03 = j02 * y, j13 = __builtin_fmaf(j12, y, -1.0f);
    const float j04 = __builtin_fmaf(-j02, x, 1.0f), j14 = -j03;
    const float j05 = -y * iz, j15 = x * iz;
    float Ja[6], Jb[6];
    Ja[0] = e2 * iz;
    Ja[1] = e3 * iz;
    Ja[2] = __builtin_fmaf(e2, j02, e3 * j12);
    Ja[3] = __builtin_fmaf(e2, j03, e3 * j13);
    Ja[4] = __builtin_fmaf(e2, j04, e3 * j14);
    Ja[5] = __builtin_fmaf(e2, j05, e3 * j15);
    Jb[0] = e4 * iz;
    Jb[1] = e5 * iz;
    Jb[2] = __builtin_fmaf(e4, j02, __builtin_fmaf(e5, j12, -1.0f));
    Jb[3] = __builtin_fmaf(e4, j03, __builtin_fmaf(e5, j13, -y));
    Jb[4] = __builtin_fmaf(e4, j04, __builtin_fmaf(e5, j14, x));
    Jb[5] = __builtin_fmaf(e4, j05, e5 * j15);
    if (lane < 3) {
      double *o = sh_delta[lane];
      const float a0 = (j & 1) ? sh_r0[n_tail - 1] : r0, a1 = (j & 1) ? sh_r1[n_tail - 1] : r1;
      o[0] = dw * (double)(a0 * a0), o[1] = dw * (double)(a0 * a1), o[2] = dw * (double)(a1 * a1);
      double *acc = o + 3;
      int t = 0;
#pragma unroll
      for (int i = 0; i < 6; ++i) {
#pragma unroll
        for (int c = i; c < 6; ++c, ++t) {
          acc[kAccAA + t] = dw * ((double)Ja[i] * (double)Ja[c]);
          acc[kAccAB + t] = dw * ((double)Ja[i] * (double)Jb[c] + (double)Jb[i] * (double)Ja[c]);
          acc[kAccBB + t] = dw * ((double)Jb[i] * (double)Jb[c]);
        }
        acc[kAccAR0 + i] = dw * ((double)Ja[i] * (double)r0);
        acc[kAccAR1 + i] = dw * ((double)Ja[i] * (double)r1);
        acc[kAccBR0 + i] = dw * ((double)Jb[i] * (double)r0);
        acc[kAccBR1 + i] = dw * ((double)Jb[i] * (double)r1);
      }
    }
  }
// ... 855 lines not shown
                                                   int h, int any_rule, int *__restrict__ kept) {
  const int x = blockIdx.x * blockDim.x + threadIdx.x, y = blockIdx.y;
  bool keep = false;
  if (x < w && y < h) {
    const unsigned char *r0 = mp + (size_t)(2 * y) * wp + 2 * x;
    const unsigned a = *(const unsigned short *)r0, b = *(const unsigned short *)(r0 + wp);
    keep = any_rule ? (a | b) != 0u : (a & b) == 0x0101u;
    mo[(size_t)y * w + x] = keep ? 1 : 0;
  }
  const unsigned long long m = __ballot(keep);
  if ((threadIdx.x & (kWave - 1)) == 0 && m) atomicAdd(kept, __popcll(m));
}

hipError_t launch_mask_plane(const unsigned char *src, int stride, unsigned char *dst, int w, int h, int *kept, hipStream_t stream) {
  LaunchGuard guard;
  hipLaunchKernelGGL(k_mask_plane, dim3((unsigned)((w + 255) / 256), (unsigned)h), dim3(256), 0, stream, src, stride, dst, w, h, kept);
  return hipGetLastError();
}

hipError_t launch_mask_down(const unsigned char *m_prev, int w_prev, unsigned char *m_out, int w, int h, int any_rule, int *kept,
                            hipStream_t stream) {
  LaunchGuard guard;
  hipLaunchKernelGGL(k_mask_down, dim3((unsigned)((w + 255) / 256), (unsigned)h), dim3(256), 0, stream, m_prev, w_prev, m_out, w, h,
                     any_rule, kept);
  return hipGetLastError();
}


template <int N>
__device__ __forceinline__ void residual_mask_pixels(const LevelPairDesc &d, const float *kt, const float *P, const float max_distance,
                                                     const float (&z_in)[N], const float (&zx)[N], const float (&zy)[N],
                                                     const float (&ri_in)[N], const float (&tx)[N], const float ty, int (&cls)[N],
                                                     float (&dist)[N]) {
  float x[N], y[N], z[N], ri[N];
#pragma unroll
  for (int k = 0; k < N; ++k) z[k] = z_in[k], ri[k] = ri_in[k], x[k] = tx[k] * z[k], y[k] = ty * z[k];
#pragma unroll
  for (int k = 0; k < N; ++k) { DVO_OPAQUE(x[k]); DVO_OPAQUE(y[k]); DVO_OPAQUE(z[k]); DVO_OPAQUE(ri[k]); }
  round_toward_zero();
#pragma unroll
  for (int k = 0; k < N; ++k) { DVO_OPAQUE(x[k]); DVO_OPAQUE(y[k]); DVO_OPAQUE(z[k]); DVO_OPAQUE(ri[k]); }
  float r0[N], r1[N];
  bool ok[N];
  {
    Proj p[N];
    Gathered g[N];
#pragma unroll
    for (int k = 0; k < N; ++k) p[k] = project_pixel_rtz<0>(kt, d, x[k], y[k], z[k]);
#pragma unroll
    for (int k = 0; k < N; ++k) g[k] = gather_pixel(d, p[k].base);
#pragma unroll
    for (int k = 0; k < N; ++k) {
      float e2, e3, e4, e5;
      finish_pixel_rtz<true>(d, p[k], g[k], z[k], ri[k], 0.0f, 0.0f, r0[k], r1[k], e2, e3, e4, e5, ok[k]);
    }
  }
#pragma unroll
  for (int k = 0; k < N; ++k) { DVO_OPAQUE(r0[k]); DVO_OPAQUE(r1[k]); }
  round_to_nearest();
#pragma unroll
  for (int k = 0; k < N; ++k) { DVO_OPAQUE(r0[k]); DVO_OPAQUE(r1[k]); }
#pragma unroll
  for (int k = 0; k < N; ++k) {
    const bool evaluated = (z_in[k] == z_in[k]) && (zx[k] == zx[k]) && (zy[k] == zy[k]);
    const float t0 = r0[k] * P[0] + r1[k] * P[1];
    const float t1 = r0[k] * P[2] + r1[k] * P[3];
    const float dd = t0 * r0[k] + t1 * r1[k];
    const bool valid = evaluated && ok[k];
    cls[k] = !evaluated ? -1 : !ok[k] ? (int)kRmInvalid : dd <= max_distance ? (int)kRmInlier : (int)kRmOutlier;
    dist[k] = valid ? dd : u2f(0x7fc00000u);
  }
}

__device__ __forceinline__ LevelPairDesc residual_mask_desc(const CurLevelDesc *cur) {
  const DVO_CONST CurLevelDesc *c = (const DVO_CONST CurLevelDesc *)cur;
  LevelPairDesc d = {};
  d.c_a = c->c_a, d.c_b = c->c_b;
  d.w = c->w, d.h = c->h;
#pragma unroll
  for (int i = 0; i < 6; ++i) d.wc[i] = c->wc[i];
#pragma unroll
  for (int i = 0; i < 4; ++i) d.wr[i] = c->wr[i];
  d.ub_x = c->ub_x, d.ub_y = c->ub_y;
  return d;
}

__global__ void __launch_bounds__(kResidualMaskBlock) k_residual_mask(const ResidualMaskRecord *__restrict__ records, int n_records) {
  constexpr int kWaves = kResidualMaskBlock / kWave, kLanePixels = kResidualMaskLanePixels;
  constexpr int kCnt = 6;
  __shared__ unsigned s_cnt[kWaves][kCnt];
  const int lane = threadIdx.x & (kWave - 1), wave = threadIdx.x >> 6;
  for (int rec = blockIdx.y; rec < n_records; rec += gridDim.y) {
    const ResidualMaskRecord R = records[rec];
    if (blockIdx.x * kResidualMaskChunk >= R.n) continue;
    const LevelPairDesc d = residual_mask_desc(R.cur);
    float kt[12];
#pragma unroll
    for (int i = 0; i < 12; ++i) kt[i] = R.kt[i];
    const int p0 = (blockIdx.x * kResidualMaskBlock + threadIdx.x) * kLanePixels;
    const bool live = p0 < R.n;
    const float qnan = u2f(0x7fc00000u);
    float z[kLanePixels] = {qnan, qnan, qnan, qnan}, zx[kLanePixels] = {qnan, qnan, qnan, qnan}, zy[kLanePixels] = {qnan, qnan, qnan, qnan};
    float ri[kLanePixels] = {0.f, 0.f, 0.f, 0.f}, tx[kLanePixels] = {0.f, 0.f, 0.f, 0.f};
    float ty = 0.f;
    if (live) {
      const float4 z4 = *(const float4 *)(R.z + p0), i4 = *(const float4 *)(R.ri + p0);
      const float4 za = *(const float4 *)(R.zd + p0), zb = *(const float4 *)(R.zd + p0 + 2);
// ... 201 lines not shown
  int c = 0;
  for (int b = b0; b < b1; ++b) c += block_partials[b].x;
  __shared__ int sh[256];
  sh[threadIdx.x] = c;
  __syncthreads();
  if (threadIdx.x == 0) {
    int run = 0;
    for (int t = 0; t < 256; ++t) {
      const int v = sh[t];
      sh[t] = run, run += v;
    }
  }
  __syncthreads();
  int run = sh[threadIdx.x];
  for (int b = b0; b < b1; ++b) prefix[b] = run, run += block_partials[b].x;
}

__global__ __launch_bounds__(256) void k_compact(const float *__restrict__ zsel, const float *__restrict__ r_i, const float *__restrict__ r_ix,
                                                 const float *__restrict__ r_iy, const float *__restrict__ tx, const float *__restrict__ ty,
                                                 int w, int n, int n_pad, const int *__restrict__ prefix, const int *__restrict__ counters,
                                                 float *__restrict__ cz, float *__restrict__ ci, float *__restrict__ cix,
                                                 float *__restrict__ ciy, float *__restrict__ ctx, float *__restrict__ cty,
                                                 int *__restrict__ cpix) {
  const int i = blockIdx.x * blockDim.x + threadIdx.x;
  const int n_pts = counters[0] & ~1;
  const float z = i < n ? zsel[i] : u2f(0x7fc00000u);
  const bool ok = z == z;
  const unsigned long long m = __ballot(ok);
  const int lane = threadIdx.x & (kWave - 1), wave = threadIdx.x >> 6;
  __shared__ int sh_cnt[4];
  if (lane == 0) sh_cnt[wave] = __popcll(m);
  __syncthreads();
  int before = prefix[blockIdx.x];
  for (int k = 0; k < wave; ++k) before += sh_cnt[k];
  if (ok) {
    const int p = before + (int)__builtin_amdgcn_mbcnt_hi((unsigned)(m >> 32), __builtin_amdgcn_mbcnt_lo((unsigned)m, 0u));
    const int row = i / w, col = i - row * w;
    cz[p] = z, ci[p] = r_i[i], cix[p] = r_ix[i], ciy[p] = r_iy[i], ctx[p] = tx[col], cty[p] = ty[row], cpix[p] = i;
  }
  if (i >= n_pts && i < n_pad) cz[i] = u2f(0x7fc00000u), ci[i] = 0.0f, cix[i] = 0.0f, ciy[i] = 0.0f, ctx[i] = 0.0f, cty[i] = 0.0f, cpix[i] = -1;
}

hipError_t launch_compact(const float *zsel, const float *r_i, const float *r_ix, const float *r_iy, const float *tx, const float *ty, int w,
                          int n, int n_pad, const int2 *block_partials, int *prefix, const int *counters, float *cz, float *ci, float *cix,
                          float *ciy, float *ctx, float *cty, int *cpix, hipStream_t stream) {
  LaunchGuard guard;
  const int n_blocks = (n_pad + 255) / 256;
  hipLaunchKernelGGL(k_select_prefix, dim3(1), dim3(256), 0, stream, block_partials, n_blocks, prefix);
  hipLaunchKernelGGL(k_compact, dim3((unsigned)n_blocks), dim3(256), 0, stream, zsel, r_i, r_ix, r_iy, tx, ty, w, n, n_pad,
                     (const int *)prefix, counters, cz, ci, cix, ciy, ctx, cty, cpix);
  return hipGetLastError();
}

__global__ void k_copy_strided(const float *__restrict__ src, int stride, float *__restrict__ dst, int w, int h) {
  const int x = blockIdx.x * blockDim.x + threadIdx.x, y = blockIdx.y;
  if (x < w && y < h) dst[(size_t)y * w + x] = src[(size_t)y * stride + x];
}

hipError_t launch_copy_strided(const float *src, int stride, float *dst, int w, int h, hipStream_t stream) {
  LaunchGuard guard;
  hipLaunchKernelGGL(k_copy_strided, dim3((unsigned)((w + 255) / 256), (unsigned)h), dim3(256), 0, stream, src, stride, dst, w,
                     h);
  return hipGetLastError();
}

template <bool kDepth>
__global__ void k_ingest(const unsigned char *__restrict__ img, int channels, int img_stride_bytes,
                         const unsigned short *__restrict__ raw_z, int z_stride, float z_scale, float *__restrict__ i_plane,
                         float *__restrict__ z_plane, int w, int h) {
  const int x4 = blockIdx.x * blockDim.x + threadIdx.x, y = blockIdx.y;
  if (x4 * 4 >= w || y >= h) return;
  const unsigned char *ip = img + (size_t)y * img_stride_bytes + (size_t)x4 * 4 * channels;
  unsigned char px[12];
  const int nb = 4 * channels;
  if ((((size_t)ip) & 3) == 0) {
    const unsigned *ip4 = (const unsigned *)ip;
#pragma unroll
    for (int k = 0; k < 3; ++k)
      if (k < channels) {
        const unsigned v = ip4[k];
        px[4 * k] = (unsigned char)v, px[4 * k + 1] = (unsigned char)(v >> 8), px[4 * k + 2] = (unsigned char)(v >> 16),
               px[4 * k + 3] = (unsigned char)(v >> 24);
      }
  } else {
#pragma unroll
    for (int k = 0; k < 12; ++k)
      if (k < nb) px[k] = ip[k];
  }
  float g[4];
#pragma unroll
  for (int k = 0; k < 4; ++k) {
    if (channels == 3) {
      const int b = px[3 * k], gg = px[3 * k + 1], r = px[3 * k + 2];
      g[k] = (float)((b * 1868 + gg * 9617 + r * 4899 + (1 << 13)) >> 14);
    } else {
      g[k] = (float)px[k];
    }
  }
  const size_t o = (size_t)y * w + (size_t)x4 * 4;
  if (!kDepth) {
    *(float4 *)(i_plane + o) = make_float4(g[0], g[1], g[2], g[3]);
    return;
  }
  const unsigned short *zp = raw_z + (size_t)y * z_stride + (size_t)x4 * 4;
  unsigned short zr[4];
  if ((((size_t)zp) & 7) == 0) {
// ... 570 lines not shown
```

dvo_slam_amd/csrc/dvo_pyramid.cpp:

```cpp
#include <dlfcn.h>
#include <emmintrin.h>

#include <algorithm>
#include <cfloat>
#include <chrono>
#include <cmath>
#include <cstdio>
#include <cstdlib>
#include <cstring>

#include "dvo_internal.h"

namespace dvo_amd {
namespace host {

constexpr size_t kDescEntryBytes = 1024;
constexpr size_t kDescChunkEntries = 256;
constexpr size_t kRefDesc0Offset = 640;
struct DeviceState {
  std::mutex mu;
  hipStream_t prep_stream = nullptr;
  std::vector<std::pair<size_t, void *>> free_slabs;
  std::vector<void *> desc_chunks, desc_free;
  std::atomic<bool> timing{false};
  hipEvent_t ev[2] = {nullptr, nullptr};
  double last_ms = 0.0;
  void *batch_area = nullptr;
  size_t batch_bytes = 0;
  int batch_launches = 0, batch_copies = 0, batch_syncs = 0;
};
DeviceState g_dev[kMaxDevices];

int device_prep_stream(int device, hipStream_t *s) {
  DeviceState &d = g_dev[device];
  std::lock_guard<std::mutex> lk(d.mu);
  if (!d.prep_stream) HIP_TRY(hipStreamCreateWithFlags(&d.prep_stream, hipStreamNonBlocking));
  *s = d.prep_stream;
  return DVO_AMD_OK;
}

std::mutex &device_mutex(int device) { return g_dev[device].mu; }

int ingest_timing(int device, int enable, double *last_ms) {
  DeviceState &d = g_dev[device];
  std::lock_guard<std::mutex> lk(d.mu);
  if (enable && !d.ev[0]) {
    HIP_TRY(hipSetDevice(device));
    for (hipEvent_t &e : d.ev) HIP_TRY(hipEventCreate(&e));
  }
  d.timing = enable != 0;
  if (last_ms) *last_ms = d.last_ms;
  return DVO_AMD_OK;
}

int slab_alloc(int device, size_t bytes, void **out) {
  DeviceState &d = g_dev[device];
  {
    std::lock_guard<std::mutex> lk(d.mu);
    for (size_t i = 0; i < d.free_slabs.size(); ++i)
      if (d.free_slabs[i].first == bytes) {
        *out = d.free_slabs[i].second;
        d.free_slabs.erase(d.free_slabs.begin() + (long)i);
        return DVO_AMD_OK;
      }
  }
  HIP_TRY(hipMalloc(out, bytes));
  return DVO_AMD_OK;
}

// ... 239 lines not shown
      desc_free(p->device, s.desc_entry);
      return fail_hip("selection planes", em);
    }
    s.extra_bytes = bytes;
    s.ref_desc = (RefLevelDesc *)s.desc_entry;
    size_t off = 0;
    for (int l = 0; l < p->n_levels; ++l) {
      s.zsel[l] = (float *)((char *)s.extra_slab + off);
      s.pts[l] = compact_at((char *)s.extra_slab + off + sizeof(float) * p->lv[l].n_pad, p->lv[l].n_pad);
      off += align_up((sizeof(float) + kCompactBytesPerPoint) * p->lv[l].n_pad, 256);
    }
  }
  auto fail = [&](const char *what, hipError_t e) {
    (void)hipStreamSynchronize(st);
    if (s.extra_slab) (void)hipFree(s.extra_slab);
    desc_free(p->device, s.desc_entry);
    return fail_hip(what, e);
  };
  RefLevelDesc ref_host[DVO_AMD_MAX_LEVELS];
  ref_level_descs(p, s, ref_host);
  DeviceState &dev = g_dev[p->device];
  const bool timed = dev.timing.load();
  hipError_t e = timed ? hipEventRecord(dev.ev[0], st) : hipSuccess;
  if (e != hipSuccess) return fail("ingest timing", e);
  e = hipMemcpyAsync(s.ref_desc, ref_host, sizeof(RefLevelDesc) * p->n_levels, hipMemcpyHostToDevice, st);
  if (e != hipSuccess) return fail("selection descriptors", e);
  for (int l = 0; l < p->n_levels; ++l) {
    const LevelData &L = p->lv[l];
    e = mask ? launch_select_masked(L.z_plane, L.c_a, L.c_b, mask->plane[l], L.n, L.n_pad, ti, td, s.zsel[l], p->counters + 2 * l,
                                    p->sel_partials, st)
             : launch_select(L.z_plane, L.c_a, L.c_b, L.n, L.n_pad, ti, td, s.zsel[l], p->counters + 2 * l, p->sel_partials, st);
    if (e != hipSuccess) return fail("select", e);
    e = launch_compact(s.zsel[l], L.r_i, L.r_ix, L.r_iy, L.tx, L.ty, L.w, L.n, L.n_pad, p->sel_partials, p->sel_prefix, p->counters + 2 * l,
                       s.pts[l].z, s.pts[l].i, s.pts[l].ix, s.pts[l].iy, s.pts[l].tx, s.pts[l].ty, s.pts[l].pix, st);
    if (e != hipSuccess) return fail("compact", e);
  }
  int host_counters[2 * DVO_AMD_MAX_LEVELS];
  e = hipMemcpyAsync(host_counters, p->counters, sizeof(int) * 2 * p->n_levels, hipMemcpyDeviceToHost, st);
  if (e != hipSuccess) return fail("selection counters", e);
  if (timed && (e = hipEventRecord(dev.ev[1], st)) != hipSuccess) return fail("ingest timing", e);
  e = hipStreamSynchronize(st);
  if (e != hipSuccess) return fail("selection", e);
  if (timed) {
    float ms = 0.f;
    if (hipEventElapsedTime(&ms, dev.ev[0], dev.ev[1]) == hipSuccess) dev.last_ms = ms;
  }
  for (int l = 0; l < p->n_levels; ++l) s.count[l] = host_counters[2 * l], s.n_pts[l] = s.count[l] & ~1, s.last[l] = host_counters[2 * l + 1];
  p->selections.push_back(std::move(sp));
  *out = p->selections.back().get();
  return DVO_AMD_OK;
}



static BatchLevel batch_level(const dvo_amd_pyramid *p, int l) {
  const LevelData &L = p->lv[l];
  const char *base = (const char *)p->slab;
  auto off = [&](const void *q) { return (size_t)((const char *)q - base); };
  BatchLevel B;
  B.i_plane = off(L.i_plane), B.z_plane = off(L.z_plane), B.c_a = off(L.c_a), B.c_b = off(L.c_b);
  B.r_i = off(L.r_i), B.r_ix = off(L.r_ix), B.r_iy = off(L.r_iy), B.tx = off(L.tx), B.ty = off(L.ty);
  const CompactLevel c = compact_at(L.pts0, L.n_pad);
  B.zsel = off(L.zsel0);
  B.pts[0] = off(c.z), B.pts[1] = off(c.i), B.pts[2] = off(c.ix), B.pts[3] = off(c.iy), B.pts[4] = off(c.tx), B.pts[5] = off(c.ty),
  B.pts[6] = off(c.pix);
  B.counters = off(p->counters + 2 * l), B.partials = off(p->sel_partials), B.prefix = off(p->sel_prefix);
  B.w = L.w, B.h = L.h, B.n = L.n, B.n_pad = L.n_pad;
  B.fx = L.fx, B.fy = L.fy, B.ox = L.ox, B.oy = L.oy;
  return B;
}

template <typename T>
static void rebase(const T *&q, const char *base) {
  q = (const T *)((const char *)q - base);
}

static void batch_descs(dvo_amd_pyramid *p, bool with_ref, BatchDescs &D) {
  static_assert(kBatchMaxLevels == DVO_AMD_MAX_LEVELS, "BatchDescs holds a pyramid's levels");
  const char *base = (const char *)p->slab;
  cur_level_descs(p, D.cur);
  Selection s;
  selection_in_slab(p, s);
  ref_level_descs(p, s, D.ref);
  for (int l = 0; l < p->n_levels; ++l) {
    rebase(D.cur[l].c_a, base), rebase(D.cur[l].c_b, base);
    RefLevelDesc &r = D.ref[l];
    rebase(r.r_zsel, base), rebase(r.r_i, base), rebase(r.r_ix, base), rebase(r.r_iy, base), rebase(r.tx, base), rebase(r.ty, base);
  }
  D.levels = p->n_levels, D.with_ref = with_ref ? 1 : 0, D.ref_offset = (unsigned)kRefDesc0Offset;
}

int pyramid_build_batch(int device, const dvo_amd_raw_batch &b, dvo_amd_pyramid **out) {
  const int count = b.count, levels = b.levels;
  const bool with_sel = b.build_selection != 0;
  HIP_TRY(hipSetDevice(device));
  hipStream_t st;
  int rc = device_prep_stream(device, &st);
  if (rc) return rc;
  DeviceState &dev = g_dev[device];
  std::vector<dvo_amd_pyramid *> pyr;
  pyr.reserve((size_t)count);
  auto bail = [&](int code) {
    (void)hipStreamSynchronize(st);
    for (dvo_amd_pyramid *p : pyr) pyramid_discard(p);
    return code;
  };
// ... 72 lines not shown
    if (timed && (e = hipEventRecord(dev.ev[1], st)) != hipSuccess) return fail_hip("ingest timing", e);
    return DVO_AMD_OK;
  }();
  if (rc) return bail(rc);
  e = hipStreamSynchronize(st);
  if (e != hipSuccess) return bail(fail_hip("batched pyramid build", e));
  if (with_sel)
    for (int f = 0; f < count; ++f) {
      std::unique_ptr<Selection> sp(new Selection());
      Selection &s = *sp;
      s.ti = b.intensity_threshold, s.td = b.depth_threshold, s.extra_slab = nullptr, s.extra_bytes = 0;
      selection_in_slab(pyr[f], s);
      const int *c = host_counters.data() + 2 * (size_t)levels * (size_t)f;
      for (int l = 0; l < levels; ++l) s.count[l] = c[2 * l], s.n_pts[l] = s.count[l] & ~1, s.last[l] = c[2 * l + 1];
      pyr[f]->selections.push_back(std::move(sp));
    }
  {
    std::lock_guard<std::mutex> lk(dev.mu);
    float ms = 0.f;
    if (timed && hipEventElapsedTime(&ms, dev.ev[0], dev.ev[1]) == hipSuccess) dev.last_ms = ms;
    dev.batch_launches = launches, dev.batch_copies = copies, dev.batch_syncs = 1;
  }
  for (int f = 0; f < count; ++f) out[f] = pyr[f];
  return DVO_AMD_OK;
}

int batch_build_stats(int device, int *kernel_launches, int *copies, int *synchronisations) {
  DeviceState &d = g_dev[device];
  std::lock_guard<std::mutex> lk(d.mu);
  if (kernel_launches) *kernel_launches = d.batch_launches;
  if (copies) *copies = d.batch_copies;
  if (synchronisations) *synchronisations = d.batch_syncs;
  return DVO_AMD_OK;
}

}
}

using namespace dvo_amd;
using namespace dvo_amd::host;

extern "C" {

void dvo_amd_pyramid_retain(dvo_amd_pyramid *p) {
  if (p) p->refs.fetch_add(1);
}

void dvo_amd_pyramid_release(dvo_amd_pyramid *p) {
  if (!p) return;
  if (p->refs.fetch_sub(1) != 1) return;
  (void)hipSetDevice(p->device);
  for (auto &s : p->selections) {
    if (s->extra_slab) (void)hipFree(s->extra_slab);
    desc_free(p->device, s->desc_entry);
  }
  desc_free(p->device, p->desc_entry);
  slab_free(p->device, p->slab_bytes, p->slab);
  delete p;
}

int dvo_amd_pyramid_levels(const dvo_amd_pyramid *p) { return p ? p->n_levels : 0; }
double dvo_amd_pyramid_timestamp(const dvo_amd_pyramid *p) { return p ? p->timestamp : 0.0; }

int dvo_amd_pyramid_level_info(const dvo_amd_pyramid *p, int level, int *width, int *height, float k[4]) {
  if (!p || level < 0 || level >= p->n_levels) return DVO_AMD_ERR_INVALID_ARGUMENT;
  const LevelData &L = p->lv[level];
  if (width) *width = L.w;
  if (height) *height = L.h;
  if (k) k[0] = L.fx, k[1] = L.fy, k[2] = L.ox, k[3] = L.oy;
  return DVO_AMD_OK;
}

int dvo_amd_pyramid_download_plane(const dvo_amd_pyramid *p, int level, int plane, float *dst) {
  if (!p || !dst || level < 0 || level >= p->n_levels || plane < 0 || plane > 5) return DVO_AMD_ERR_INVALID_ARGUMENT;
  HIP_TRY(hipSetDevice(p->device));
  hipStream_t st;
  int rc = device_prep_stream(p->device, &st);
  if (rc) return rc;
  const LevelData &L = p->lv[level];
  float *tmp = nullptr;
  HIP_TRY(hipMalloc((void **)&tmp, sizeof(float) * L.n));
  hipError_t e = launch_unpack_plane(L.c_a, L.c_b, plane, L.n, tmp, st);
  if (e == hipSuccess) e = hipMemcpyAsync(dst, tmp, sizeof(float) * L.n, hipMemcpyDeviceToHost, st);
  if (e == hipSuccess) e = hipStreamSynchronize(st);
  (void)hipFree(tmp);
  if (e != hipSuccess) return fail_hip("download_plane", e);
  return DVO_AMD_OK;
}

static int select_entry(dvo_amd_pyramid *p, int level, float ti, float td, const dvo_amd_mask *sel_mask, int *count, unsigned char *mask) {
  if (!p || level < 0 || level >= p->n_levels) return DVO_AMD_ERR_INVALID_ARGUMENT;
  const Selection *sp = nullptr;
  int rc = pyramid_selection(p, ti, td, sel_mask, &sp);
  if (rc) return rc;
  const Selection &s = *sp;
  if (count) *count = s.count[level];
  if (mask) {
    HIP_TRY(hipSetDevice(p->device));
    hipStream_t st;
    rc = device_prep_stream(p->device, &st);
    if (rc) return rc;
    const LevelData &L = p->lv[level];
    unsigned char *tmp = nullptr;
    HIP_TRY(hipMalloc((void **)&tmp, L.n));
    const int dropped = (s.count[level] & 1) ? s.last[level] : -1;
    hipError_t e = launch_mask_from_zsel(s.zsel[level], L.n, dropped, tmp, st);
    if (e == hipSuccess) e = hipMemcpyAsync(mask, tmp, L.n, hipMemcpyDeviceToHost, st);
    if (e == hipSuccess) e = hipStreamSynchronize(st);
    (void)hipFree(tmp);
    if (e != hipSuccess) return fail_hip("select mask", e);
  }
  return DVO_AMD_OK;
}

int dvo_amd_pyramid_select(dvo_amd_pyramid *p, int level, float ti, float td, int *count, unsigned char *mask) {
  return select_entry(p, level, ti, td, nullptr, count, mask);
}

int dvo_amd_pyramid_select_masked(dvo_amd_pyramid *p, int level, float ti, float td, const dvo_amd_mask *mask, int *count,
                                  unsigned char *out_mask) {
  return select_entry(p, level, ti, td, mask, count, out_mask);
}

}
```

dvo_slam_amd/csrc/dvo_tracker.cpp:

```cpp
#include <dlfcn.h>
#include <emmintrin.h>

#include <algorithm>
#include <cfloat>
#include <chrono>
#include <cmath>
#include <cstdio>
#include <cstdlib>
#include <cstring>

#include "dvo_internal.h"

namespace dvo_amd {
namespace host {

thread_local std::string g_last_error;

int fail_hip(const char *what, hipError_t e) {
  g_last_error = std::string(what) + ": " + hipGetErrorString(e);
  return e == hipErrorOutOfMemory ? DVO_AMD_ERR_OUT_OF_MEMORY : DVO_AMD_ERR_HIP;
}

dvo_amd_iteration_stats *stats_push(Job &j) {
  dvo_amd_result *r = j.result;
// ... 468 lines not shown
inline double now_ns() {
  return (double)std::chrono::duration_cast<std::chrono::nanoseconds>(std::chrono::steady_clock::now().time_since_epoch()).count();
}

int submit_tick(dvo_amd_context *ctx, std::vector<Job> &jobs, GroupTick &grp) {
  const double t_begin = ctx->host_prof ? now_ns() : 0.0;
  grp.in_flight = false;
  int active_pairs = 0;
  for (size_t ji = grp.lo; ji < grp.hi; ++ji) active_pairs += jobs[ji].done ? 0 : 1;
  const bool speculate_levels = ctx->spec_levels == 1 || (ctx->spec_levels < 0 && active_pairs <= kSpecLevelsMaxPairs);
  auto wants_spec = [&](const Job &j) {
    return speculate_levels && j.have_a && !j.have_b && !j.a.cont && j.level > j.cfg->last_level;
  };
  const unsigned seq = ctx->tick_seq = next_seq(ctx->tick_seq);
  grp.seq = seq;

  std::vector<TickItem> items;
  std::vector<FinItem> fin_items;
  items.reserve(grp.hi - grp.lo);
  fin_items.reserve(grp.hi - grp.lo);
  for (size_t ji = grp.lo; ji < grp.hi; ++ji) {
    Job &j = jobs[ji];
    if (j.done) continue;
    j.sub_ll = j.sub_res = false;
    if (!j.have_a && !j.have_b) continue;
    const size_t slot_index = (size_t)(j.slot - ctx->slots.data());
    TickItem w;
    std::memset(&w, 0, sizeof(w));
    int res_steps = 1, ll_steps = 1;
    w.ref = j.sel->ref_desc + j.level;
    w.cur = j.cur->cur_desc + j.level;
    w.slot = ctx->slot_desc + slot_index;
    FinItem f;
    std::memset(&f, 0, sizeof(f));
    f.ll_partials = j.slot->ll_partials;
    f.seg_prefix_out = j.slot->seg_prefix[0], f.out = j.slot->out, f.out_dev = nullptr, f.seq = seq;
    f.ll_qmax_off = j.slot->ll_qmax_off;
    if (j.have_b) {
      j.b.steps = level_steps(ctx, j.ref->lv[j.level]);
      j.b.n_blocks = level_blocks(j.sel, j.level, j.b.steps);
    }
    if (j.have_a) {
      if (j.a.buf) w.flags |= kItemLlBuf;
      w.ll_cut_rank = j.a.cut_rank;
      item_set_ll_merge(w, level_ll_merge(ctx, j.a.steps));
      w.ll_level_blocks = (uint16_t)j.a.n_blocks;
      w.ll_first = 0;
      w.ll_blocks = (uint16_t)ll_blocks_total(j.a.n_blocks, item_ll_merge_log2(w));
      ll_steps = j.a.steps;
      f.n_ll_blocks = w.ll_blocks, f.ll_first = 0, f.ll_level_blocks = w.ll_level_blocks, f.ll_merge_log2 = (uint16_t)item_ll_merge_log2(w);
      j.sub_ll = true;
    }
    if (j.have_b) {
      w.res_blocks = (uint16_t)j.b.n_blocks;
      res_steps = j.b.steps;
      if (j.b.buf) w.flags |= kItemResBuf;
      if (j.b.k == 0) w.flags |= kItemUnitWeights;
      make_kt(j.cur->lv[j.level], j.b.estimate_after, w.kt);
      f.records = j.slot->records;
      f.n_blocks = w.res_blocks, f.level_blocks = w.res_blocks;
      f.seg_prefix_out = j.slot->seg_prefix[j.b.buf];
      if (ctx->rcp.table && j.b.k != 0) f.q7_off256 = (uint16_t)ctx->q7_off256;
      j.sub_res = true;
      j.sub_px = (double)j.sel->count[j.level];
      j.result->n_residual_passes++;
      j.alg_px += j.sub_px;
    } else if (wants_spec(j)) {
      const int nl = j.level - 1;
      speculate_next_level(j, j.spec_b);
      j.spec_b.steps = level_steps(ctx, j.ref->lv[nl]);
      j.spec_b.n_blocks = level_blocks(j.sel, nl, j.spec_b.steps);
      w.ref = j.sel->ref_desc + nl;
      w.cur = j.cur->cur_desc + nl;
      w.res_blocks = (uint16_t)j.spec_b.n_blocks;
      res_steps = j.spec_b.steps;
      if (j.spec_b.buf) w.flags |= kItemResBuf;
      w.flags |= kItemUnitWeights;
      make_kt(j.cur->lv[nl], j.spec_b.estimate_after, w.kt);
      f.records = j.slot->records;
      f.n_blocks = w.res_blocks, f.level_blocks = w.res_blocks;
      f.seg_prefix_out = j.slot->seg_prefix[j.spec_b.buf];
      j.have_spec = true;
      j.sub_res = true;
      j.sub_px = (double)j.sel->count[nl];
      j.result->n_residual_passes++;
      j.alg_px += j.sub_px;
    }
    std::memcpy(w.P, j.have_a ? j.a.P : j.precision, sizeof(w.P));
    item_set_steps(w, res_steps, ll_steps);
    items.push_back(w);
    fin_items.push_back(f);
    j.result->n_ticks++;
  }
  if (items.empty()) return DVO_AMD_OK;

  const size_t cap = (size_t)std::min(std::max(ctx->items_per_launch, 1), kMaxItemsPerLaunch);
  const size_t n_launch = (items.size() + cap - 1) / cap;
  const size_t per = (items.size() + n_launch - 1) / n_launch;
  size_t launch_index = 0;
  for (size_t first = 0; first < items.size(); first += per, ++launch_index) {
    hipStream_t st;
    {
      int rc = tick_stream(ctx, ctx->timing ? 0 : grp.stream_first + launch_index, &st);
      if (rc) return rc;
    }
    TickArgs ta;
    const int n_here = (int)std::min(per, items.size() - first);
    ta.n_items = n_here;
    ta.compact = 0;
    ta.rcp = ctx->rcp;
    int max_blocks = 0;
    int order[kMaxItemsPerLaunch];
    tick_items_order(items.data() + first, n_here, ctx->sort_items, ctx->share_placement, order);
    for (int i = 0; i < n_here; ++i) {
      ta.items[i] = items[first + (size_t)order[i]];
      max_blocks = std::max(max_blocks, (int)ta.items[i].res_blocks + (int)ta.items[i].ll_blocks);
    }
    size_t ev = 0;
    if (ctx->timing) {
      int rc = timing_begin(ctx, &ev);
      if (rc) return rc;
      double rb = 0, lb = 0, px = 0, res_steps = 0, ll_steps = 0;
      for (int i = 0; i < n_here; ++i) {
        rb += ta.items[i].res_blocks, lb += ta.items[i].ll_blocks;
        res_steps += (double)ta.items[i].res_blocks * kWavesPerBlock * item_res_steps(ta.items[i]);
        if (ta.items[i].ll_blocks) ll_steps += (double)ta.items[i].ll_level_blocks * kWavesPerBlock * item_ll_steps(ta.items[i]);
      }
      for (size_t ji = grp.lo, k = 0; ji < grp.hi; ++ji) {
        const Job &j = jobs[ji];
        if (j.done || !(j.sub_ll || j.sub_res)) continue;
// ... 179 lines not shown
}

int runner_fail_told(dvo_amd_context *ctx, int code) {
  (void)runner_fail(ctx, code);
  ctx->runner->unreported_failure = DVO_AMD_OK;
  return code;
}

int runner_reported_status(Runner &R, unsigned long long ticket) {
  if (ticket == 0) {
    const int st = R.unreported_failure;
    R.unreported_failure = DVO_AMD_OK;
    return st;
  }
  for (const Runner::Failure &f : R.failures)
    if (f.batch == ticket) {
      R.unreported_failure = DVO_AMD_OK;
      return f.status;
    }
  return DVO_AMD_OK;
}

int queue_must_be_idle(dvo_amd_context *ctx, const char *what) {
  if (ctx->runner && (ctx->runner->resident > 0 || !ctx->runner->pending.empty())) {
    g_last_error = std::string(what) + " while submitted pairs are still in flight (dvo_amd_match_wait first)";
    return DVO_AMD_ERR_INVALID_ARGUMENT;
  }
  return DVO_AMD_OK;
}

int runner_step(dvo_amd_context *ctx, size_t g) {
  Runner &R = *ctx->runner;
  GroupTick &grp = R.groups[g];
  const dvo_amd_config &cfg = ctx->cfg;
  int rc = complete_tick(ctx, R.jobs, grp);
  if (rc) return rc;
  for (size_t sidx = grp.lo; sidx < grp.hi; ++sidx)
    if (R.jobs[sidx].done && R.batch_of_slot[sidx] != 0) runner_finish_slot(R, sidx);
  for (size_t sidx = grp.lo; sidx < grp.hi && !R.pending.empty(); ++sidx) {
    Job &j = R.jobs[sidx];
    if (!j.done) continue;
    const Pending q = R.pending.front();
    R.pending.pop_front();
    j = Job();
    j.ref = q.ref, j.cur = q.cur;
    j.result = q.result;
    j.slot = &ctx->slots[sidx];
    j.cfg = &ctx->cfg;
    R.batch_of_slot[sidx] = q.batch;
    R.resident++;
    rc = pyramid_selection(j.ref, q.ti, q.td, q.mask, &j.sel);
    dvo_amd_mask_release(q.mask);
    if (rc) return rc;
    dvo_amd_result *r = j.result;
    r->n_levels = 0, r->n_iterations = 0, r->n_ticks = 0, r->n_residual_passes = 0, r->alg_bytes = 0.0, r->alg_bytes_discarded = 0.0, r->is_nan = 0;
    if (!r->iterations) r->iterations_capacity = 0;
    j.inc = q.has_init ? se3_from_matrix(q.T_init) : SE3::identity();
    j.initial = j.inc;
    j.estimate = SE3::identity();
    j.level = cfg.first_level;
    j.done = false;
    start_level(j);
  }
  return submit_tick(ctx, R.jobs, grp);
}

int runner_drain(dvo_amd_context *ctx) {
  Runner &R = *ctx->runner;
  while (R.resident > 0 || !R.pending.empty()) {
    const size_t g = R.next_group;
    R.next_group = (R.next_group + 1) % R.groups.size();
    int rc = runner_step(ctx, g);
    if (rc) return runner_fail_told(ctx, rc);
  }
  return DVO_AMD_OK;
}

int runner_configure(dvo_amd_context *ctx, int in_flight, int n_pad) {
  Runner &R = *ctx->runner;
  in_flight = std::max(in_flight, 1);
  const bool same = R.in_flight == in_flight && R.timing == ctx->timing && (int)ctx->slots.size() >= in_flight &&
                    ctx->slot_n_pad >= n_pad && ctx->slot_n_pad > 0;
  if (same) return DVO_AMD_OK;
  if (R.in_flight > 0) {
    int rc = runner_drain(ctx);
    if (rc) return rc;
  }
  int rc = ensure_slots(ctx, in_flight, n_pad);
  if (rc) return rc;
  R.jobs.assign((size_t)in_flight, Job());
  for (Job &j : R.jobs) j.done = true;
  R.batch_of_slot.assign((size_t)in_flight, 0ull);
  const int cap = std::min(std::max(ctx->items_per_launch, 1), kMaxItemsPerLaunch);
  const int n_groups = ctx->timing ? 1 : std::min(kMaxTickStreams, (in_flight + cap - 1) / cap);
  const int per_group = (in_flight + n_groups - 1) / n_groups;
  R.groups.assign((size_t)n_groups, GroupTick());
  for (int g = 0; g < n_groups; ++g) {
    R.groups[(size_t)g].lo = (size_t)std::min(g * per_group, in_flight);
    R.groups[(size_t)g].hi = (size_t)std::min((g + 1) * per_group, in_flight);
    R.groups[(size_t)g].stream_first = (size_t)g;
    R.groups[(size_t)g].id = g;
  }
  R.next_group = 0;
  R.in_flight = in_flight;
  R.timing = ctx->timing;
  R.resident = 0;
// ... 120 lines not shown
}

const char *dvo_amd_last_error(void) { return g_last_error.c_str(); }

int dvo_amd_device_count(void) {
  int n = 0;
  if (hipGetDeviceCount(&n) != hipSuccess) return 0;
  return n;
}

void dvo_amd_default_config(dvo_amd_config *c) {
  if (!c) return;
  c->first_level = 3;
  c->last_level = 1;
  c->max_iterations_per_level = 100;
  c->precision = 5e-7;
  c->mu = 0.0;
  c->use_initial_estimate = 0;
  c->intensity_derivative_threshold = 0.0f;
  c->depth_derivative_threshold = 0.0f;
  c->segment_geometry = DVO_AMD_GEOMETRY_THROUGHPUT;
  c->reserved = 0;
}

int dvo_amd_context_create(int device, const dvo_amd_config *cfg, dvo_amd_context **out) {
  if (!out) return DVO_AMD_ERR_INVALID_ARGUMENT;
  *out = nullptr;
  int ndev = 0;
  int rc = have_device(&ndev);
  if (rc) return rc;
  if (device < 0 || device >= ndev || device >= kMaxDevices) return DVO_AMD_ERR_INVALID_ARGUMENT;
  dvo_amd_config c;
  dvo_amd_default_config(&c);
  if (cfg) c = *cfg;
  rc = check_config(&c);
  if (rc) return rc;
  HIP_TRY(hipSetDevice(device));
  dvo_amd_context *ctx = new dvo_amd_context();
  ctx->device = device;
  ctx->cfg = c;
  hipError_t e = hipStreamCreateWithFlags(&ctx->stream, hipStreamNonBlocking);
  if (e != hipSuccess) {
    delete ctx;
    return fail_hip("hipStreamCreate", e);
  }
  const char *pe = getenv("DVO_AMD_POLL");
  ctx->poll = !(pe && pe[0] == '0');
  const char *fs = getenv("DVO_AMD_FIN_STAMPS");
  ctx->fin_stamps = fs && fs[0] == '1';
  const char *fp = getenv("DVO_AMD_FIN_PRIORITY");
  ctx->fin_priority = !(fp && fp[0] == '0');
  if (const char *so = getenv("DVO_AMD_SORT_ITEMS")) ctx->sort_items = so[0] != '0';
  if (const char *sp = getenv("DVO_AMD_SHARE_PLACEMENT")) ctx->share_placement = sp[0] == '0' ? 0 : sp[0] == '2' ? 2 : 1;
  const char *sa = getenv("DVO_AMD_SMALL_ARGS");
  ctx->small_args = !(sa && sa[0] == '0');
  const char *hp = getenv("DVO_AMD_HOST_PROF");
  ctx->host_prof = hp && hp[0] == '1';
  if (const char *sl = getenv("DVO_AMD_SPEC_LEVELS")) ctx->spec_levels = sl[0] == '1' ? 1 : 0;
  if (const char *fs2 = getenv("DVO_AMD_FAULT_SLOT_ALLOC")) ctx->fault_slot_alloc = atoi(fs2);
  if (const char *sa = getenv("DVO_AMD_LEVEL_STEPS_AT"))
    (void)sscanf(sa, "%lld,%lld,%lld,%lld,%lld", &ctx->level_steps_at[0], &ctx->level_steps_at[1], &ctx->level_steps_at[2],
                 &ctx->level_steps_at[3], &ctx->level_steps_at[4]);
  if (const char *fsx = getenv("DVO_AMD_FINE_STEPS")) ctx->fine_steps = atoi(fsx);
  if (const char *lm = getenv("DVO_AMD_LL_MERGE")) {
    const int v = atoi(lm);
    if (v == 1 || v == 2 || v == 4 || v == 8 || v == 16) ctx->ll_merge = v;
  }
  if (const char *rm = getenv("DVO_AMD_RCP"))
    if (rm[0] == 'h' || rm[0] == 'H' || rm[0] == 's' || rm[0] == 'S') {
      const int rrc = dvo_amd_set_reciprocal_mode(ctx, DVO_AMD_RCP_HOST_SSE);
      if (rrc) {
        dvo_amd_context_destroy(ctx);
        return rrc;
      }
    }
  if (const char *ipl = getenv("DVO_AMD_ITEMS_PER_LAUNCH")) {
    const int v = atoi(ipl);
    if (v >= 1 && v <= kMaxItemsPerLaunch) ctx->items_per_launch = v;
  }
  *out = ctx;
  return DVO_AMD_OK;
}

void dvo_amd_context_destroy(dvo_amd_context *ctx) {
  if (!ctx) return;
  if (ctx->host_prof && ctx->prof_ticks > 0)
    std::fprintf(stderr, "[dvo_amd host profile] ticks %lld, pair-ticks %lld: submit %.2f us/tick, wait %.2f us/tick, process %.2f us/tick "
                         "(%.2f us per pair-tick of host work)\n",
                 ctx->prof_ticks, ctx->prof_job_ticks, ctx->prof_submit_ns / ctx->prof_ticks * 1e-3,
                 ctx->prof_wait_ns / ctx->prof_ticks * 1e-3, ctx->prof_process_ns / ctx->prof_ticks * 1e-3,
                 (ctx->prof_submit_ns + ctx->prof_process_ns) / std::max(1LL, ctx->prof_job_ticks) * 1e-3);
  if (ctx->host_prof && ctx->ovf_checks > 0)
    std::fprintf(stderr, "[dvo_amd host profile] exact likelihood-overflow checks: %lld (%lld said the reference's product overflowed)\n",
                 ctx->ovf_checks, ctx->ovf_hits);
  (void)hipSetDevice(ctx->device);
  if (ctx->stream) (void)hipStreamSynchronize(ctx->stream);
  if (ctx->runner) {
    if (ctx->runner->resident > 0 || !ctx->runner->pending.empty()) (void)runner_fail(ctx, DVO_AMD_ERR_INVALID_ARGUMENT);
    delete ctx->runner;
    ctx->runner = nullptr;
  }
  dvo_amd_comm_destroy(ctx);
  dvo_amd_exchange_destroy(ctx);
  for (hipStream_t st : ctx->extra_streams) {
    (void)hipStreamSynchronize(st);
    (void)hipStreamDestroy(st);
// ... 298 lines not shown
```

dvo_slam_amd/csrc/dvo_types.h:

```cpp
#pragma once
#include <hip/hip_runtime.h>
#include <stdint.h>

namespace dvo_amd {

constexpr int kWave = 64;
constexpr int kBlockThreads = 256;
constexpr int kWavesPerBlock = kBlockThreads / kWave;
constexpr int kStepPx = kWave;
constexpr int kMaxSteps = 64;
constexpr int kPlanePad = kStepPx * kMaxSteps * kWavesPerBlock;

constexpr int kRecCount = 0, kRecFirstW = 1, kRecLastR = 2, kRecS0 = 4, kRecS1 = 7, kRecWaveCnt = 10, kRecAcc = 16;
constexpr int kNumAcc = 87;
constexpr int kRecStride = 104;
constexpr int kAccAA = 0, kAccAB = 21, kAccBB = 42, kAccAR0 = 63, kAccAR1 = 69, kAccBR0 = 75, kAccBR1 = 81;

constexpr int kLevelChunksMax = 16;
__host__ __device__ inline int level_chunks_log2(int nb) { return nb >= 128 ? 4 : nb >= 64 ? 3 : nb >= 32 ? 2 : nb >= 16 ? 1 : 0; }
__host__ __device__ inline int chunk_lo(int nb, int c) { return (nb * c) >> level_chunks_log2(nb); }
__host__ __device__ inline void leaf_range(int nb, int g_log2, int i, int *lo, int *hi) {
  const int per = g_log2 - level_chunks_log2(nb);
  const int c = i >> per, q = i & ((1 << per) - 1);
  const int c_lo = chunk_lo(nb, c), len = chunk_lo(nb, c + 1) - c_lo;
  *lo = c_lo + ((len * q) >> per), *hi = c_lo + ((len * (q + 1)) >> per);
}
__host__ __device__ inline void band_blocks(int nb, int n_bands, int b, int *first, int *count) {
  const int C = 1 << level_chunks_log2(nb);
  const int lo = chunk_lo(nb, C * b / n_bands), hi = chunk_lo(nb, C * (b + 1) / n_bands);
  *first = lo, *count = hi - lo;
}
__host__ __device__ inline int ll_chunk_blocks(int len, int m_log2) {
  const int k = (len + ((1 << m_log2) >> 1)) >> m_log2;
  return len <= 0 ? 0 : (k < 1 ? 1 : k);
}
__host__ __device__ inline int ll_blocks_before(int nb, int m_log2, int c) {
  int n = 0;
  for (int i = 0; i < c; ++i) n += ll_chunk_blocks(chunk_lo(nb, i + 1) - chunk_lo(nb, i), m_log2);
  return n;
}
__host__ __device__ inline int ll_blocks_total(int nb, int m_log2) { return ll_blocks_before(nb, m_log2, 1 << level_chunks_log2(nb)); }
__host__ __device__ inline void ll_block_range(int nb, int m_log2, int lb, int *first, int *count) {
  int before = 0;
  *first = 0, *count = 0;
  const int C = 1 << level_chunks_log2(nb);
  for (int c = 0; c < C; ++c) {
    const int lo = chunk_lo(nb, c), len = chunk_lo(nb, c + 1) - lo;
    const int here = ll_chunk_blocks(len, m_log2);
    if (lb < before + here) {
      const int j = lb - before;
      *first = lo + len * j / here;
      *count = lo + len * (j + 1) / here - *first;
      return;
    }
    before += here;
  }
}

struct RefLevelDesc {
  const float *r_zsel;
  const float *r_i, *r_ix, *r_iy;
  const float *tx, *ty;
};
struct CurLevelDesc {
  const float4 *c_a;
  const float2 *c_b;
  int w, h;
  float wc[6];
  float wr[4];
  float ub_x, ub_y;
};
struct SlotDesc {
  float2 *res[2];
  float *records;
  double *ll_partials;
  float *ll_qmax;
  int *seg_prefix[2];
  float *dbg_w;
};

struct TickItem {
  const RefLevelDesc *ref;
  const CurLevelDesc *cur;
  const SlotDesc *slot;
  uint16_t res_blocks, ll_blocks;
  uint16_t res_first, ll_first;
  uint8_t steps_log2;
  uint8_t flags;
  uint16_t ll_level_blocks;
  int ll_cut_rank;
  float kt[12];
  float P[4];
};
__host__ __device__ inline int steps_of_code(int c) {
  return c < 7 ? 1 << c : c == 7 ? 10 : c == 8 ? 20 : c == 9 ? 12 : c == 10 ? 14 : c == 11 ? 6 : c == 12 ? 18 : c == 13 ? 24 : c == 14 ? 40 : 30;
}
__host__ __device__ inline int item_res_steps(const TickItem &it) { return steps_of_code(it.steps_log2 & 15); }
__host__ __device__ inline int item_ll_steps(const TickItem &it) { return steps_of_code(it.steps_log2 >> 4); }
__host__ __device__ inline int item_ll_merge_log2(const TickItem &it) { return (it.flags >> 4) & 7; }
inline void item_set_steps(TickItem &it, int res_steps, int ll_steps) {
  auto code = [](int steps) {
    for (int c = 0; c < 16; ++c)
      if (steps_of_code(c) == steps) return c;
    int c = 0;
    while ((1 << c) < steps) ++c;
    return c;
  };
  it.steps_log2 = (uint8_t)(code(res_steps) | (code(ll_steps) << 4));
}
inline void item_set_ll_merge(TickItem &it, int merge) {
  int m = 0;
  while ((1 << m) < merge) ++m;
  it.flags = (uint8_t)((it.flags & 0x8F) | (m << 4));
}
constexpr unsigned kItemResBuf = 1;
constexpr unsigned kItemLlBuf = 2;
constexpr unsigned kItemUnitWeights = 4;
static_assert(sizeof(TickItem) == 104, "TickItem is packed to fit many items into one kernel-argument block");

constexpr int kMaxItemsPerLaunch = 62;
struct RcpTable {
  const unsigned *table;
  int shift;
  int unit;
  const unsigned *nibbles;
};
struct Q7Rec {
  double S[3];
  double acc[87];
  int n_tail, valid;
  int idx[3];
  float w_table[3];
  float w_exact[3];
  int recomputed_equal;
};
static_assert(sizeof(Q7Rec) == 768, "Q7Rec: three 256-byte lines of the slot's block");
constexpr int kRcpNibbleWordsMax = 512;
struct TickArgs {
  int n_items;
  int compact;
  RcpTable rcp;
  uint16_t group_first[kMaxItemsPerLaunch + 4];
  uint8_t xcd_rot[kMaxItemsPerLaunch + 2] = {};
  uint8_t tail_rot[kMaxItemsPerLaunch + 2] = {};
  uint8_t set_size[kMaxItemsPerLaunch + 2] = {};
  uint32_t set_inv[kMaxItemsPerLaunch] = {};
  static constexpr bool kSets = true;
  TickItem items[kMaxItemsPerLaunch];
};
static_assert(sizeof(TickArgs) <= 8192, "kernel argument block too large");

struct FinOut {
  int valid;
  int has_res;
  int has_ll;
  unsigned seq;
  double S[3];
  double S_odd[3];
  float first_w, last_r0, last_r1;
  float ll_qmax;
  double acc[kNumAcc];
  double ll_sum;
};
static_assert(sizeof(FinOut) % 16 == 0, "FinOut is copied in 16-byte pieces");

constexpr int kFinWords = (int)(sizeof(FinOut) / 4);
constexpr int kFinWirePieces = (kFinWords + 1) / 2;
struct alignas(16) FinWire {
  unsigned piece[kFinWirePieces][4];
};
// ... 60 lines not shown
};
struct FinArgsSmall {
  int n_items;
  int pad;
  FinItem items[kMaxSmallItems];
};

hipError_t launch_tick(const TickArgs &args, int max_blocks, hipStream_t stream, hipEvent_t t_start = nullptr,
                       hipEvent_t t_stop = nullptr);
int tick_args_layout(TickArgs &args, int max_blocks, int share = 0);
int tick_args_layout(TickArgsSmall &args, int max_blocks);
void tick_items_order(const TickItem *items, int n, bool sort, int share, int *order);
int tick_args_locate(const TickArgs &args, unsigned block, int *bx);
hipError_t launch_tick_small(const TickArgsSmall &args, int max_blocks, hipStream_t stream, hipEvent_t t_start = nullptr,
                             hipEvent_t t_stop = nullptr);
hipError_t launch_finalize_small(const FinArgsSmall &args, hipStream_t stream);
typedef Q7ArgsT<kMaxSmallItems> Q7ArgsSmall;
hipError_t launch_q7_tail(const Q7Args &args, hipStream_t stream);
hipError_t launch_q7_tail_small(const Q7ArgsSmall &args, hipStream_t stream);
hipError_t launch_finalize(const FinArgs &args, hipStream_t stream);
hipError_t launch_ll_overflow(const float2 *res, const int *seg_prefix, int seg_first, int n_segs, int seg_px, int rank_offset,
                              int n_px, int cut_rank, int rank_end, const float P[4], unsigned *result_host, hipStream_t stream);
hipError_t launch_exchange_record(const FinOut *rec_dev, const struct ExchangeArgs *exchange_dev, unsigned xseq, hipStream_t stream);
constexpr float kLlOverflowScreen = 7.0e6f;
hipError_t read_finalize_stamps(unsigned long long out[8]);
long long read_block_trace(unsigned long long *out, long long capacity);
hipError_t launch_rcp_table_probe(const RcpTable &rcp, const float *in, float *out, int n, hipStream_t stream);
hipError_t launch_rcp_midpoint_probe(int k, unsigned *out_rn, unsigned *out_rtz, hipStream_t stream);

hipError_t launch_marker(unsigned tag, hipStream_t stream);
hipError_t launch_queue_probe(unsigned *out_pinned, hipStream_t stream);
int acc_mode();

hipError_t launch_pyr_down(const float *i_prev, const float *z_prev, int w_prev, float *i_out, float *z_out, int w, int h,
                           hipStream_t stream);
hipError_t launch_level_planes(const float *i_plane, const float *z_plane, int w, int h, int n_pad, float fx, float fy,
                               float ox, float oy, float4 *c_a, float2 *c_b, float *r_i, float *r_ix, float *r_iy,
                               float *tx, float *ty, int ty_len, hipStream_t stream);
hipError_t launch_select(const float *z_plane, const float4 *c_a, const float2 *c_b, int n, int n_pad, float ti, float td,
                         float *zsel, int *counters, int2 *block_partials, hipStream_t stream);
hipError_t launch_select_masked(const float *z_plane, const float4 *c_a, const float2 *c_b, const unsigned char *mask, int n, int n_pad,
                                float ti, float td, float *zsel, int *counters, int2 *block_partials, hipStream_t stream);
hipError_t launch_mask_plane(const unsigned char *src, int stride, unsigned char *dst, int w, int h, int *kept, hipStream_t stream);
hipError_t launch_mask_down(const unsigned char *m_prev, int w_prev, unsigned char *m_out, int w, int h, int any_rule, int *kept,
                            hipStream_t stream);
hipError_t launch_ingest(const unsigned char *img, int channels, int img_stride_bytes, const unsigned short *raw_z,
                         int z_stride, float z_scale, float *i_plane, float *z_plane, int w, int h, hipStream_t stream);
hipError_t launch_ingest_intensity(const unsigned char *img, int channels, int img_stride_bytes, float *i_plane, int w, int h,
                                   hipStream_t stream);
hipError_t launch_copy_strided(const float *src, int stride, float *dst, int w, int h, hipStream_t stream);
hipError_t launch_compact(const float *zsel, const float *r_i, const float *r_ix, const float *r_iy, const float *tx, const float *ty, int w,
                          int n, int n_pad, const int2 *block_partials, int *prefix, const int *counters, float *cz, float *ci, float *cix,
                          float *ciy, float *ctx, float *cty, int *cpix, hipStream_t stream);
hipError_t launch_mask_from_zsel(const float *zsel, int n, int last_dropped, unsigned char *mask, hipStream_t stream);
hipError_t launch_unpack_plane(const float4 *c_a, const float2 *c_b, int plane, int n, float *dst, hipStream_t stream);

struct BatchFrame {
  char *slab;
  char *desc;
  const unsigned char *img;
  const unsigned short *z;
};
struct BatchLevel {
  size_t i_plane, z_plane, c_a, c_b, r_i, r_ix, r_iy, tx, ty;
  size_t zsel, pts[7];
  size_t counters, partials, prefix;
  int w, h, n, n_pad;
  float fx, fy, ox, oy;
};
constexpr int kBatchMaxLevels = 8;
struct BatchDescs {
  CurLevelDesc cur[kBatchMaxLevels];
  RefLevelDesc ref[kBatchMaxLevels];
  int levels, with_ref;
  unsigned ref_offset;
};
hipError_t launch_ingest_batch(const BatchFrame *frames, int count, int channels, int img_stride_bytes, int z_stride, float z_scale,
                               const BatchLevel &L0, hipStream_t stream, int *launches);
hipError_t launch_pyr_down_batch(const BatchFrame *frames, int count, const BatchLevel &prev, const BatchLevel &L, hipStream_t stream,
                                 int *launches);
hipError_t launch_level_planes_batch(const BatchFrame *frames, int count, const BatchLevel &L, hipStream_t stream, int *launches);
hipError_t launch_batch_descs(const BatchFrame *frames, int count, const BatchDescs &descs, hipStream_t stream, int *launches);
hipError_t launch_select_batch(const BatchFrame *frames, int count, const BatchLevel &L, float ti, float td, int *all_counters,
                               int level, int levels, hipStream_t stream, int *launches);
hipError_t launch_compact_batch(const BatchFrame *frames, int count, const BatchLevel &L, hipStream_t stream, int *launches);

constexpr int kResidualMaskBlock = 256;
constexpr int kResidualMaskLanePixels = 4;
constexpr int kResidualMaskChunk = kResidualMaskBlock * kResidualMaskLanePixels;
enum { kRmEvaluated = 0, kRmInvalid, kRmInlier, kRmOutlier, kRmLast, kRmDone, kRmWords = 8 };
struct ResidualMaskRecord {
  const float *z;
  const float2 *zd;
  const float *ri;
  const float *tx, *ty;
  const CurLevelDesc *cur;
  unsigned char *out;
  float *distance;
  int *kept;
  unsigned *counts;
  int w, n;
  float kt[12];
  float P[4];
  float max_distance;
  int invalid_keep, unevaluated_keep;
};
// ... 38 lines not shown
```

include/dvo_amd_debug.h:

```cpp
#ifndef DVO_AMD_DEBUG_H_
#define DVO_AMD_DEBUG_H_

#include "dvo_amd.h"

#ifdef __cplusplus
extern "C" {
#endif

long long dvo_amd_debug_block_trace(dvo_amd_context *ctx, unsigned long long *out, long long capacity_blocks);
int dvo_amd_debug_rcp(dvo_amd_context *ctx, int n, const float *in, float *out);

int dvo_amd_debug_combine_bands(int n_bands, const double *bands, double *out);
unsigned dvo_amd_debug_next_seq(unsigned seq);
int dvo_amd_debug_wire_layout(int *n_pieces, int *n_record_words);
int dvo_amd_debug_take_wire(const unsigned *wire, unsigned tick, int from_piece, unsigned *record_words);
int dvo_amd_debug_tick_layout(int n_items, const int *res_blocks, const int *ll_blocks, const int *res_steps, const int *ref_key,
                              const int *cur_key, int share, int max_blocks, int *order, int *group_first, int *xcd_rot,
                              int *tail_rot, int *set_size, int *compact, int *n_blocks, long long capacity_blocks, int *block_item,
                              int *block_index);

typedef struct {
  int valid_constraints;
  int reserved;
  double scale_sums[3];
  float scale[4];
  float precision[4];
  double moments[87];
  double information[36];
  double rhs[6];
  double loglik_sum;
  float loglik;
  float reserved_f;
} dvo_amd_iteration_probe;
int dvo_amd_debug_iteration(dvo_amd_context *ctx, dvo_amd_pyramid *reference, dvo_amd_pyramid *current, int level,
                            const float *T, const float *precision_in, const float *precision_eval,
                            dvo_amd_iteration_probe *out);

typedef struct {
  int n_tail;
  int valid_constraints;
  int valid_counted;
  int recomputed_equal;
  int pixel[3];
  float weight_table[3];
  float weight_exact[3];
  double scale_sums_delta[3];
  double moments_delta[87];
} dvo_amd_q7_probe;
int dvo_amd_debug_weights(dvo_amd_context *ctx, dvo_amd_pyramid *reference, dvo_amd_pyramid *current, int level, const float *T,
                          const float *precision_in, float *weights, dvo_amd_q7_probe *tail);

int dvo_amd_debug_residuals_masked(dvo_amd_context *ctx, dvo_amd_pyramid *reference, dvo_amd_pyramid *current, int level, const float *T,
                             const dvo_amd_mask *mask, float *residuals, int *n_valid);
int dvo_amd_debug_iteration_masked(dvo_amd_context *ctx, dvo_amd_pyramid *reference, dvo_amd_pyramid *current, int level,
                                   const float *T, const float *precision_in, const float *precision_eval,
                                   const dvo_amd_mask *mask, dvo_amd_iteration_probe *out);
int dvo_amd_debug_weights_masked(dvo_amd_context *ctx, dvo_amd_pyramid *reference, dvo_amd_pyramid *current, int level,
                                 const float *T, const float *precision_in, const dvo_amd_mask *mask, float *weights,
                                 dvo_amd_q7_probe *tail);

int dvo_amd_debug_hw_queue(dvo_amd_context *ctx, int *pipe_queue);

int dvo_amd_debug_level_geometry(dvo_amd_context *ctx, dvo_amd_pyramid *reference, int level, int *steps, int *blocks, int *points);

int dvo_amd_bench_residual_pass(dvo_amd_context *ctx, dvo_amd_pyramid *reference, dvo_amd_pyramid *current, int level,
                                const float *T, int n_items, int rounds, int reps, double *avg_ms, double *alg_bytes,
                                int *n_launches);

int dvo_amd_bench_residual_pass_pairs(dvo_amd_context *ctx, int n_items, dvo_amd_pyramid *const *references,
                                      dvo_amd_pyramid *const *currents, int level, const float *T, int rounds, int reps,
                                      double *avg_ms, double *alg_bytes, int *n_launches);

int dvo_amd_debug_finalize_stamps(dvo_amd_context *ctx, unsigned long long *stamps8);

int dvo_amd_debug_tick_log(dvo_amd_context *ctx, double *out, int capacity_records, int *n_records);

int dvo_amd_kernel_timing(dvo_amd_context *ctx, int enable, double *ms_residual_pass, long long *n_launches, int reset);

int dvo_amd_debug_rcp_form(const dvo_amd_context *ctx, int *form, char *note, int note_capacity);

int dvo_amd_debug_marker(dvo_amd_context *ctx, unsigned tag);

int dvo_amd_debug_ll_overflow(dvo_amd_context *ctx, const float *residuals, int n_blocks, int steps, int seg_first, int n_segs,
                              int rank_offset, int rank_end, int cut_rank, const float *precision, int *overflowed);

int dvo_amd_debug_map_timing(dvo_amd_context *ctx, double *device_ms, double *copy_ms, long long *points);
int dvo_amd_debug_covisibility_ms(const dvo_amd_context *ctx, double *device_ms);
int dvo_amd_debug_keyframe_map_timing(const dvo_amd_map *map, double *device_ms, double *copy_ms, long long *delta_points,
                                      long long *delta_voxels, int *merge_tile);
int dvo_amd_debug_map_merge(dvo_amd_context *ctx, long long na, const unsigned long long *keys_a, const unsigned long long *acc_a,
                            long long nb, const unsigned long long *keys_b, const unsigned long long *acc_b,
                            unsigned long long *keys_out, unsigned long long *acc_out, long long *n_out);
int dvo_amd_debug_graph_timing(dvo_amd_context *ctx, double *linearise_ms, double *factorize_ms, int *n_padded,
                               int *factorizations);
int dvo_amd_debug_graph_batch_records(dvo_amd_context *ctx, int graph, int capacity, dvo_amd_graph_iteration *records,
                                      int *n_recorded);
int dvo_amd_debug_graph_system(dvo_amd_context *ctx, int n_vertices, const double *poses, const int *fixed, int n_edges,
                               const dvo_amd_graph_edge *edges, double robust_delta, double *H, double *b, double *x,
                               double *F, int *n_free, int *failed_pivot);
int dvo_amd_debug_graph_system_sparse(dvo_amd_context *ctx, int n_vertices, const double *poses, const int *fixed,
                                      int n_edges, const dvo_amd_graph_edge *edges, double robust_delta, int block_capacity,
                                      int *n_blocks, int *block_rc, double *blocks, double *b, double *x, double *F,
                                      int *n_free, int *failed_pivot);
int dvo_amd_debug_graph_symbolic(int n_vertices, const int *fixed, int n_edges, const dvo_amd_graph_edge *edges,
                                 int capacity, int *n_free, int *n_fronts, int *n_update, int *n_levels, int *widest,
                                 int *perm, int *parent, int *level, int *pivot_ptr, int *pivot, int *update_ptr, int *update,
                                 double *factor_doubles, double *flops);
int dvo_amd_debug_graph_sparse_timing(dvo_amd_context *ctx, double *symbolic_ms, double *linearise_ms, double *factorize_ms,
                                      double *solve_ms, int *fronts, int *levels, int *widest, double *factor_doubles,
                                      double *flops);
int dvo_amd_debug_ingest_timing(int device, int enable, double *last_ms);
int dvo_amd_debug_batch_build_stats(int device, int *kernel_launches, int *copies, int *synchronisations);
// ... 15 lines not shown
```

Before: 63240.

## Precompute per-point float4 records for reference points in residual pass

Adds a per-selection build step that packs the compacted reference point arrays into two float4 records (z, x, y, 1/z and intensity, gradients, occlusion threshold), computed once and cached on the selection. When enabled per level, the residual pass reads two 16-byte vector loads instead of six scalar loads and skips the back-projection, reciprocal and occlusion-threshold arithmetic per pixel per iteration. This raises the bytes read per point and adds a one-time build with host synchronisations and extra device memory. Levels where derived values are not finite fall back to the original path.

```diff
diff --git a/dvo_slam_amd/capi.py b/dvo_slam_amd/capi.py
--- a/dvo_slam_amd/capi.py
+++ b/dvo_slam_amd/capi.py
@@ -65,6 +65,7 @@
     "dvo_amd_default_warp_options", "dvo_amd_warp_inverse", "dvo_amd_warp_inverse_many", "dvo_amd_pyramid_warp_inverse",
     "dvo_amd_pyramid_warp_inverse_many", "dvo_amd_warp_forward", "dvo_amd_warp_forward_many", "dvo_amd_pyramid_warp_forward",
     "dvo_amd_pyramid_warp_forward_many", "dvo_amd_debug_warp_timing",
+    "dvo_amd_debug_point_records",
     "dvo_amd_default_volume_options", "dvo_amd_default_volume_raycast_options", "dvo_amd_volume_create", "dvo_amd_volume_destroy",
     "dvo_amd_volume_clear", "dvo_amd_volume_options_get", "dvo_amd_volume_integrate", "dvo_amd_volume_insert",
     "dvo_amd_volume_set_poses", "dvo_amd_volume_remove", "dvo_amd_volume_stats", "dvo_amd_volume_download", "dvo_amd_volume_raycast",
@@ -494,6 +495,9 @@
     L.dvo_amd_mask_info.argtypes = [vp, ip, ip, ip, C.POINTER(C.c_longlong)]
     L.dvo_amd_mask_download.argtypes = [vp, C.c_int, C.POINTER(C.c_ubyte)]
     L.dvo_amd_pyramid_select_masked.argtypes = [vp, C.c_int, C.c_float, C.c_float, vp, C.POINTER(C.c_int), C.POINTER(C.c_ubyte)]
+    if hasattr(L, "dvo_amd_debug_point_records"):
+        L.dvo_amd_debug_point_records.argtypes = [vp, vp, C.c_float, C.c_float, C.c_int, C.c_int, fp, fp, fp, C.POINTER(C.c_int),
+                                                  C.POINTER(C.c_int), C.POINTER(C.c_int)]
     L.dvo_amd_match_masked.argtypes = [vp, vp, vp, C.c_float, C.c_float, vp, dp, C.POINTER(CResult)]
     L.dvo_amd_match_many_masked.argtypes = [vp, C.c_int, C.POINTER(vp), C.POINTER(vp), C.POINTER(vp), dp, C.POINTER(CResult), C.c_int]
     L.dvo_amd_default_budget_options.argtypes = [C.POINTER(BudgetOptions)]
@@ -1617,6 +1621,19 @@
                                             out.ctypes.data_as(C.POINTER(C.c_ubyte))), "pyramid_select")
         return cnt.value, out
 
+    def point_records(self, level: int, ti: float = 0.0, td: float = 0.0, mask: "SelectionMask | None" = None):
+        n, n_points, in_use = C.c_int(), C.c_int(), C.c_int()
+        m = None if mask is None else mask._h
+        _check(lib().dvo_amd_debug_point_records(self._h, m, ti, td, level, 0, None, None, None, C.byref(n), C.byref(n_points),
+                                                 C.byref(in_use)), "dvo_amd_debug_point_records")
+        rec_a, rec_b = np.empty((n.value, 4), np.float32), np.empty((n.value, 4), np.float32)
+        plain = np.empty((6, n.value), np.float32)
+        _check(lib().dvo_amd_debug_point_records(self._h, m, ti, td, level, n.value, _fp(rec_a), _fp(rec_b), _fp(plain), C.byref(n),
+                                                 C.byref(n_points), C.byref(in_use)), "dvo_amd_debug_point_records")
+        out = dict(rec_a=rec_a, rec_b=rec_b, n_points=n_points.value, in_use=bool(in_use.value))
+        out.update({name: plain[k] for k, name in enumerate(("z", "i", "ix", "iy", "tx", "ty"))})
+        return out
+
 
     def fuse_depth(self, frames, transformations, options=None, counts: bool = False, observations: bool = False):
         got = RgbdImagePyramid.fuse_depth_many([self], [frames], [transformations], options, counts=counts, observations=observations)
diff --git a/dvo_slam_amd/csrc/dvo_internal.h b/dvo_slam_amd/csrc/dvo_internal.h
--- a/dvo_slam_amd/csrc/dvo_internal.h
+++ b/dvo_slam_amd/csrc/dvo_internal.h
@@ -80,6 +80,11 @@
   void *desc_entry = nullptr;
   void *extra_slab;
   size_t extra_bytes;
+  mutable bool rec_built = false;
+  mutable unsigned rec_levels = 0;
+  mutable void *rec_slab = nullptr;
+  mutable size_t rec_bytes = 0;
+  mutable float4 *rec_a[DVO_AMD_MAX_LEVELS] = {}, *rec_b[DVO_AMD_MAX_LEVELS] = {};
 };
 
 struct LevelData {
@@ -252,6 +257,7 @@
   bool fin_stamps = false;
   bool sort_items = true;
   int share_placement = 1;
+  bool point_records = true;
   bool fin_priority = true;
   bool small_args = true;
   bool poll = true;
@@ -292,6 +298,7 @@
 struct Job {
   dvo_amd_pyramid *ref = nullptr, *cur = nullptr;
   const Selection *sel = nullptr;
+  unsigned rec_levels = 0;
   dvo_amd_result *result = nullptr;
   JobSlot *slot = nullptr;
   const dvo_amd_config *cfg = nullptr;
@@ -378,6 +385,7 @@
 inline int pyramid_selection(dvo_amd_pyramid *p, float ti, float td, const Selection **out) {
   return pyramid_selection(p, ti, td, nullptr, out);
 }
+int selection_point_records(dvo_amd_pyramid *p, const Selection *s, unsigned *levels);
 int mask_fits(const char *entry, const dvo_amd_pyramid *p, const dvo_amd_mask *mask);
 std::mutex &device_mutex(int device);
 int pyramid_build(int device, const PyramidSpec &spec, const Level0Source &src, dvo_amd_pyramid **out);
diff --git a/dvo_slam_amd/csrc/dvo_kernels.hip b/dvo_slam_amd/csrc/dvo_kernels.hip
--- a/dvo_slam_amd/csrc/dvo_kernels.hip
+++ b/dvo_slam_amd/csrc/dvo_kernels.hip
@@ -112,6 +112,7 @@
 
 struct LevelPairDesc {
   const float *r_zsel, *r_i, *r_ix, *r_iy, *tx, *ty;
+  const float4 *rec_a, *rec_b;
   const float4 *c_a;
   const float2 *c_b;
   float2 *res[2];
@@ -188,8 +189,14 @@
   return __builtin_nontemporal_load(p);
 }
 
+__device__ __forceinline__ float occlusion_threshold_rtz(float z) {
+  float s = z - 0.4f;
+  s = 0.0012f + (0.0019f * s) * s;
+  return -20.0f * s;
+}
+
 template <bool ZERO_E>
-__device__ __forceinline__ void finish_pixel_rtz(const LevelPairDesc &d, const Proj &p, const Gathered &g, float z, float ri,
+__device__ __forceinline__ void finish_pixel_rtz(const LevelPairDesc &d, const Proj &p, const Gathered &g, float thr, float ri,
                                                  float rix, float riy, float &r0, float &r1, float &e2, float &e3, float &e4,
                                                  float &e5, bool &valid) {
   const float w1u = __builtin_amdgcn_fractf(p.u), w1v = __builtin_amdgcn_fractf(p.v);
@@ -205,9 +212,7 @@
   const bool has_nan = __builtin_isunordered(ci, cz) || __builtin_isunordered(cix, ciy) || __builtin_isunordered(czx, czy);
   const float t0 = d.wc[0] * ci + d.wr[0] * ri;
   const float t1 = d.wc[1] * cz + d.wr[1] * p.sz;
-  float s = z - 0.4f;
-  s = 0.0012f + (0.0019f * s) * s;
-  valid = p.inb && !has_nan && (t1 > -20.0f * s);
+  valid = p.inb && !has_nan && (t1 > thr);
   r0 = valid ? t0 : 0.0f;
   r1 = valid ? t1 : 0.0f;
   e2 = d.wc[2] * cix + d.wr[2] * rix;
@@ -235,20 +240,44 @@
 #endif
 #define DVO_KEEP(x) asm volatile("" ::"v"(x))
 
+constexpr int kResidualKBufs = 2;
 template <int ACC, int RCP>
+struct ResidualLds {
+  static __device__ __forceinline__ unsigned *rcp() {
+    __shared__ unsigned rcp_lds[RCP == 2 ? kRcpNibbleWordsMax : 1];
+    return rcp_lds;
+  }
+  static __device__ __forceinline__ float *stage() {
+    __shared__ __attribute__((aligned(16))) float stage[ACC >= 1 ? kWavesPerBlock * kResidualKBufs * kWave * 16 : 4];
+    return stage;
+  }
+  static __device__ __forceinline__ v2f (*pair_slots())[kWave + 2] {
+    __shared__ __attribute__((aligned(8))) v2f pair_slots[kWavesPerBlock][kWave + 2];
+    return pair_slots;
+  }
+  static __device__ __forceinline__ float (*sums())[kRecStride] {
+    __shared__ float sm[kWavesPerBlock][kRecStride];
+    return sm;
+  }
+};
+
+template <int ACC, int RCP, int REC>
 __device__ void residual_pass(const TickItem &it, const LevelPairDesc &d_in, const int lb) {
+  static_assert(REC == 0 || ACC >= 1, "the register-accumulator form reads the plain arrays");
   LevelPairDesc d = d_in;
-  __shared__ unsigned rcp_lds[RCP == 2 ? kRcpNibbleWordsMax : 1];
+  unsigned *const rcp_lds = ResidualLds<ACC, RCP>::rcp();
   if (RCP == 2) {
     const int words = (1 << (23 - d.rcp.shift)) >> 3;
     for (int i = threadIdx.x; i < words; i += kBlockThreads) rcp_lds[i] = ((const DVO_GLOBAL unsigned *)d.rcp.nibbles)[i];
     __syncthreads();
     d.rcp_lds = rcp_lds;
   }
-  constexpr int kBufs = 2;
-  const int lane = threadIdx.x & (kWave - 1);
-  const int wave = threadIdx.x >> 6;
-  const int wave_s = __builtin_amdgcn_readfirstlane(wave);
+  constexpr int kBufs = kResidualKBufs;
+  const int wave_s = __builtin_amdgcn_readfirstlane((int)(threadIdx.x >> 6));
+  int lane_v = threadIdx.x & (kWave - 1);
+  if (REC) asm volatile("" : "+v"(lane_v));
+  const int lane = lane_v;
+  const int wave = REC ? wave_s : (int)(threadIdx.x >> 6);
   const int seg = lb * kWavesPerBlock + wave;
   const int steps = item_res_steps(it);
   unsigned idx = (unsigned)(seg * (kStepPx * steps) + lane);
@@ -260,12 +289,11 @@
   v4acc gram_p[kGramPairs];
 #pragma unroll
   for (int k = 0; k < kGramPairs; ++k) gram_p[k] = v4acc{0.0f, 0.0f, 0.0f, 0.0f};
-  __shared__ __attribute__((aligned(16))) float stage[ACC >= 1 ? kWavesPerBlock * kBufs * kWave * 16 : 4];
+  float *const stage = ResidualLds<ACC, RCP>::stage();
   float S0[3] = {0.0f, 0.0f, 0.0f}, S1[3] = {0.0f, 0.0f, 0.0f};
   float first_w = 0.0f;
   int run_count = 0;
-  __shared__ __attribute__((aligned(8))) v2f pair_slots[kWavesPerBlock][kWave + 2];
-  v2f *const slots = pair_slots[wave];
+  v2f *const slots = ResidualLds<ACC, RCP>::pair_slots()[wave];
   if (lane == 0) slots[0] = v2f{0.0f, 0.0f};
 
   float kt[12];
@@ -282,12 +310,18 @@
   const DVO_GLOBAL void *const p_z = (const DVO_GLOBAL void *)d.r_zsel, *const p_i = (const DVO_GLOBAL void *)d.r_i,
                          *const p_ix = (const DVO_GLOBAL void *)d.r_ix, *const p_iy = (const DVO_GLOBAL void *)d.r_iy,
                          *const p_tx = (const DVO_GLOBAL void *)d.tx, *const p_ty = (const DVO_GLOBAL void *)d.ty;
+  const DVO_GLOBAL void *const p_ra = (const DVO_GLOBAL void *)d.rec_a, *const p_rb = (const DVO_GLOBAL void *)d.rec_b;
   DVO_GLOBAL char *const p_res = (DVO_GLOBAL char *)((it.flags & kItemResBuf) ? d.res[1] : d.res[0]);
 
   float n_z, n_i, n_ix, n_iy, n_tx, n_ty;
+  v4f n_a, n_b;
   auto load_first = [&](const bool opaque) __attribute__((always_inline)) {
     unsigned at = idx;
     if (opaque) DVO_OPAQUE(at);
+    if (REC) {
+      n_a = ld_off<v4f>(p_ra, 16u * at), n_b = ld_off<v4f>(p_rb, 16u * at);
+      return;
+    }
     n_z = ld_off<float>(p_z, 4u * at), n_i = ld_off<float>(p_i, 4u * at), n_ix = ld_off<float>(p_ix, 4u * at),
     n_iy = ld_off<float>(p_iy, 4u * at);
     n_tx = ld_off<float>(p_tx, 4u * at), n_ty = ld_off<float>(p_ty, 4u * at);
@@ -327,12 +361,19 @@
     }
   };
 
-  auto do_step = [&](const int step, const int q, const bool prefetch) __attribute__((always_inline)) {
+  auto do_step = [&](const int step, const int q, const bool prefetch, const bool stay = false) __attribute__((always_inline)) {
     const unsigned cur_idx = idx;
-    float z = n_z, ri = n_i, rix = n_ix, riy = n_iy;
-    float x = n_tx * z, y = n_ty * z;
+    float z = REC ? n_a.x : n_z, ri = REC ? n_b.x : n_i, rix = REC ? n_b.y : n_ix, riy = REC ? n_b.z : n_iy;
+    float x = REC ? n_a.y : n_tx * z, y = REC ? n_a.z : n_ty * z;
+    const float rec_iz = REC ? n_a.w : 0.0f;
+    const float rec_thr = REC ? n_b.w : 0.0f;
     idx += kWave;
     auto prefetch_next = [&]() __attribute__((always_inline)) {
+      if (REC) {
+        const unsigned at = stay ? cur_idx : idx;
+        n_a = ld_off<v4f>(p_ra, 16u * at), n_b = ld_off<v4f>(p_rb, 16u * at);
+        return;
+      }
       n_z = ld_off<float>(p_z, 4u * idx), n_i = ld_off<float>(p_i, 4u * idx), n_ix = ld_off<float>(p_ix, 4u * idx),
       n_iy = ld_off<float>(p_iy, 4u * idx);
       n_tx = ld_off<float>(p_tx, 4u * idx), n_ty = ld_off<float>(p_ty, 4u * idx);
@@ -360,13 +401,15 @@
         __builtin_amdgcn_sched_barrier(0);
       }
       if (prefetch) prefetch_next();
-      finish_pixel_rtz<ACC == 0>(d, p, g, z, ri, rix, riy, r0, r1, e2, e3, e4, e5, ok);
+      finish_pixel_rtz<ACC == 0>(d, p, g, REC ? rec_thr : occlusion_threshold_rtz(z), ri, rix, riy, r0, r1, e2, e3, e4, e5, ok);
     }
     DVO_OPAQUE(r0); DVO_OPAQUE(r1); DVO_OPAQUE(e2); DVO_OPAQUE(e3); DVO_OPAQUE(e4); DVO_OPAQUE(e5);
-    DVO_OPAQUE(x); DVO_OPAQUE(y); DVO_OPAQUE(z);
+    DVO_OPAQUE(x); DVO_OPAQUE(y);
+    if (!REC) DVO_OPAQUE(z);
     round_to_nearest();
     DVO_OPAQUE(r0); DVO_OPAQUE(r1); DVO_OPAQUE(e2); DVO_OPAQUE(e3); DVO_OPAQUE(e4); DVO_OPAQUE(e5);
-    DVO_OPAQUE(x); DVO_OPAQUE(y); DVO_OPAQUE(z);
+    DVO_OPAQUE(x); DVO_OPAQUE(y);
+    if (!REC) DVO_OPAQUE(z);
 
     {
       const float qnan = u2f(0x7fc00000u);
@@ -392,8 +435,8 @@
     wgt = ok ? wgt : 0.0f;
     if (RCP && d.dbg_w) ((DVO_GLOBAL float *)d.dbg_w)[cur_idx] = ok ? wgt : u2f(0x7fc00000u);
 
-    x = ok ? x : 0.0f, y = ok ? y : 0.0f, z = ok ? z : 1.0f;
-    const float iz = __builtin_amdgcn_rcpf(z);
+    if (!REC) x = ok ? x : 0.0f, y = ok ? y : 0.0f, z = ok ? z : 1.0f;
+    const float iz = REC ? rec_iz : __builtin_amdgcn_rcpf(z);
     const float iz2 = iz * iz;
     const float j02 = -x * iz2, j12 = -y * iz2;
     const float j03 = j02 * y, j13 = __builtin_fmaf(j12, y, -1.0f);
@@ -500,6 +543,12 @@
       bool marked = false;
 #endif
       load_first(false);
+      if (REC) {
+        for (int step = 0; step < steps; step += 2) {
+          do_step(step, 0, true);
+          do_step(step + 1, 1, true, step + 2 >= steps);
+        }
+      } else {
       for (int step = 0; step + 2 < steps; step += 2) {
         do_step(step, 0, true);
 #if defined(DVO_TRACE_BLOCKS) && !defined(DVO_TRACE_DESC)
@@ -513,6 +562,7 @@
       if (!marked && threadIdx.x == 0) trace_first = trace_clock();
 #endif
       do_step(steps - 1, 1, false);
+      }
     }
   }
 
@@ -524,7 +574,7 @@
   }
   if (ACC >= 1 && !(DVO_ABLATE & 1) && steps > 0) gram_from_stage(1);
 
-  __shared__ float sm[kWavesPerBlock][kRecStride];
+  float(*const sm)[kRecStride] = ResidualLds<ACC, RCP>::sums();
   if (ACC == 0) {
 #pragma unroll
     for (int i = 0; i < kNumAcc; ++i) {
@@ -569,7 +619,7 @@
       sm[wave][kRecLastR + 1] = last.y;
     }
   }
-  const int tid = threadIdx.x;
+  const int tid = REC ? wave_s * kWave + lane : (int)threadIdx.x;
   int e0 = 0, e1 = -1;
   if (ACC >= 1 && tid < kNumAcc) {
     if (tid < kAccAR0) {
@@ -824,6 +874,7 @@
   LevelPairDesc d;
   d.r_zsel = r->r_zsel, d.r_i = r->r_i, d.r_ix = r->r_ix, d.r_iy = r->r_iy;
   d.tx = r->tx, d.ty = r->ty;
+  d.rec_a = r->rec_a, d.rec_b = r->rec_b;
   d.c_a = c->c_a, d.c_b = c->c_b;
   d.w = c->w, d.h = c->h;
 #pragma unroll
@@ -857,9 +908,12 @@
   d.rcp = rcp;
   d.rcp_lds = nullptr;
   d.dbg_w = RCP ? ((const DVO_CONST SlotDesc *)it.slot)->dbg_w : nullptr;
-  if (bx < rb)
-    residual_pass<ACC, RCP>(it, d, it.res_first + xcd_contiguous_block(bx, rb));
-  else
+  if (bx < rb) {
+    if (ACC >= 1 && (it.flags & kItemPointRecords))
+      residual_pass<ACC, RCP, ACC >= 1>(it, d, it.res_first + xcd_contiguous_block(bx, rb));
+    else
+      residual_pass<ACC, RCP, 0>(it, d, it.res_first + xcd_contiguous_block(bx, rb));
+  } else
     loglik_pass(it, d, (int)it.ll_first + (bx - rb));
 #ifdef DVO_TRACE_BLOCKS
   if (threadIdx.x == 0) {
@@ -995,7 +1049,7 @@
     {
       const Proj p = project_pixel_rtz<1>(kt, d, x, y, z);
       const Gathered g = gather_pixel(d, p.base);
-      finish_pixel_rtz<true>(d, p, g, z, ri, rix, riy, r0, r1, e2, e3, e4, e5, ok);
+      finish_pixel_rtz<true>(d, p, g, occlusion_threshold_rtz(z), ri, rix, riy, r0, r1, e2, e3, e4, e5, ok);
     }
     DVO_OPAQUE(r0); DVO_OPAQUE(r1); DVO_OPAQUE(e2); DVO_OPAQUE(e3); DVO_OPAQUE(e4); DVO_OPAQUE(e5);
     DVO_OPAQUE(x); DVO_OPAQUE(y); DVO_OPAQUE(z);
@@ -1957,7 +2011,7 @@
 #pragma unroll
     for (int k = 0; k < N; ++k) {
       float e2, e3, e4, e5;
-      finish_pixel_rtz<true>(d, p[k], g[k], z[k], ri[k], 0.0f, 0.0f, r0[k], r1[k], e2, e3, e4, e5, ok[k]);
+      finish_pixel_rtz<true>(d, p[k], g[k], occlusion_threshold_rtz(z[k]), ri[k], 0.0f, 0.0f, r0[k], r1[k], e2, e3, e4, e5, ok[k]);
     }
   }
 #pragma unroll
@@ -2265,6 +2319,47 @@
   return hipGetLastError();
 }
 
+__global__ __launch_bounds__(256) void k_point_records(const float *__restrict__ cz, const float *__restrict__ ci,
+                                                       const float *__restrict__ cix, const float *__restrict__ ciy,
+                                                       const float *__restrict__ ctx, const float *__restrict__ cty, int n_pad,
+                                                       v4f *__restrict__ rec_a, v4f *__restrict__ rec_b, int *__restrict__ not_finite) {
+  const int p = blockIdx.x * blockDim.x + threadIdx.x;
+  if (p >= n_pad) return;
+  float z = cz[p];
+  DVO_OPAQUE(z);
+  round_toward_zero();
+  DVO_OPAQUE(z);
+  float thr = occlusion_threshold_rtz(z);
+  DVO_OPAQUE(thr); DVO_OPAQUE(z);
+  round_to_nearest();
+  DVO_OPAQUE(thr); DVO_OPAQUE(z);
+  const bool pad = !(z == z);
+  const float x = pad ? 0.0f : ctx[p] * z, y = pad ? 0.0f : cty[p] * z;
+  const float iz = pad ? 1.0f : __builtin_amdgcn_rcpf(z);
+  {
+    const float iz2 = iz * iz;
+    const float j02 = -x * iz2, j12 = -y * iz2;
+    const float j03 = j02 * y, j13 = __builtin_fmaf(j12, y, -1.0f);
+    const float j04 = __builtin_fmaf(-j02, x, 1.0f);
+    const float j05 = -y * iz, j15 = x * iz;
+    const float t[12] = {x, y, iz, iz2, j02, j12, j03, j13, j04, j05, j15, 0.0f};
+    bool finite = true;
+#pragma unroll
+    for (int k = 0; k < 12; ++k) finite = finite && __builtin_fabsf(t[k]) < __builtin_inff();
+    if (!finite) atomicAdd(not_finite, 1);
+  }
+  rec_a[p] = v4f{z, x, y, iz};
+  rec_b[p] = v4f{ci[p], cix[p], ciy[p], thr};
+}
+
+hipError_t launch_point_records(const float *cz, const float *ci, const float *cix, const float *ciy, const float *ctx, const float *cty,
+                                int n_pad, float4 *rec_a, float4 *rec_b, int *not_finite, hipStream_t stream) {
+  LaunchGuard guard;
+  hipLaunchKernelGGL(k_point_records, dim3((unsigned)((n_pad + 255) / 256)), dim3(256), 0, stream, cz, ci, cix, ciy, ctx, cty, n_pad,
+                     (v4f *)rec_a, (v4f *)rec_b, not_finite);
+  return hipGetLastError();
+}
+
 __global__ void k_copy_strided(const float *__restrict__ src, int stride, float *__restrict__ dst, int w, int h) {
   const int x = blockIdx.x * blockDim.x + threadIdx.x, y = blockIdx.y;
   if (x < w && y < h) dst[(size_t)y * w + x] = src[(size_t)y * stride + x];
diff --git a/dvo_slam_amd/csrc/dvo_pyramid.cpp b/dvo_slam_amd/csrc/dvo_pyramid.cpp
--- a/dvo_slam_amd/csrc/dvo_pyramid.cpp
+++ b/dvo_slam_amd/csrc/dvo_pyramid.cpp
@@ -14,7 +14,7 @@
 namespace dvo_amd {
 namespace host {
 
-constexpr size_t kDescEntryBytes = 1024;
+constexpr size_t kDescEntryBytes = 1280;
 constexpr size_t kDescChunkEntries = 256;
 constexpr size_t kRefDesc0Offset = 640;
 struct DeviceState {
@@ -360,6 +360,62 @@
 }
 
 
+int selection_point_records(dvo_amd_pyramid *p, const Selection *sel, unsigned *levels) {
+  std::lock_guard<std::mutex> lk(p->mu);
+  const Selection &s = *sel;
+  *levels = 0;
+  if (s.rec_built) {
+    *levels = s.rec_levels;
+    return DVO_AMD_OK;
+  }
+  HIP_TRY(hipSetDevice(p->device));
+  hipStream_t st;
+  int rc = device_prep_stream(p->device, &st);
+  if (rc) return rc;
+  size_t bytes = 0;
+  for (int l = 0; l < p->n_levels; ++l) bytes += 2 * align_up(sizeof(float4) * (size_t)p->lv[l].n_pad, 256);
+  const size_t counters_at = bytes;
+  bytes += align_up(sizeof(int) * DVO_AMD_MAX_LEVELS, 256);
+  void *slab = nullptr;
+  rc = slab_alloc(p->device, bytes, &slab);
+  if (rc) return rc;
+  int *const counters = (int *)((char *)slab + counters_at);
+  float4 *ra[DVO_AMD_MAX_LEVELS] = {}, *rb[DVO_AMD_MAX_LEVELS] = {};
+  const float4 *ptrs[DVO_AMD_MAX_LEVELS][2];
+  int not_finite[DVO_AMD_MAX_LEVELS] = {};
+  size_t off = 0;
+  hipError_t e = hipMemsetAsync(counters, 0, sizeof(int) * DVO_AMD_MAX_LEVELS, st);
+  for (int l = 0; l < p->n_levels && e == hipSuccess; ++l) {
+    const size_t one = align_up(sizeof(float4) * (size_t)p->lv[l].n_pad, 256);
+    ra[l] = (float4 *)((char *)slab + off), rb[l] = (float4 *)((char *)slab + off + one);
+    off += 2 * one;
+    const CompactLevel &c = s.pts[l];
+    e = launch_point_records(c.z, c.i, c.ix, c.iy, c.tx, c.ty, p->lv[l].n_pad, ra[l], rb[l], counters + l, st);
+  }
+  if (e == hipSuccess) e = hipMemcpyAsync(not_finite, counters, sizeof(int) * p->n_levels, hipMemcpyDeviceToHost, st);
+  if (e == hipSuccess) e = hipStreamSynchronize(st);
+  unsigned ok_levels = 0;
+  if (e == hipSuccess) {
+    for (int l = 0; l < p->n_levels; ++l) {
+      const bool ok = not_finite[l] == 0;
+      ptrs[l][0] = ok ? ra[l] : nullptr, ptrs[l][1] = ok ? rb[l] : nullptr;
+      if (ok) ok_levels |= 1u << l;
+    }
+    e = hipMemcpy2DAsync((char *)s.ref_desc + offsetof(RefLevelDesc, rec_a), sizeof(RefLevelDesc), ptrs, sizeof(ptrs[0]), sizeof(ptrs[0]),
+                         (size_t)p->n_levels, hipMemcpyHostToDevice, st);
+    if (e == hipSuccess) e = hipStreamSynchronize(st);
+  }
+  if (e != hipSuccess) {
+    (void)hipStreamSynchronize(st);
+    slab_free(p->device, bytes, slab);
+    return fail_hip("point records", e);
+  }
+  for (int l = 0; l < p->n_levels; ++l) s.rec_a[l] = ra[l], s.rec_b[l] = rb[l];
+  s.rec_slab = slab, s.rec_bytes = bytes, s.rec_levels = ok_levels, s.rec_built = true;
+  *levels = ok_levels;
+  return DVO_AMD_OK;
+}
+
 
 static BatchLevel batch_level(const dvo_amd_pyramid *p, int l) {
   const LevelData &L = p->lv[l];
@@ -538,6 +594,7 @@
   (void)hipSetDevice(p->device);
   for (auto &s : p->selections) {
     if (s->extra_slab) (void)hipFree(s->extra_slab);
+    if (s->rec_slab) slab_free(p->device, s->rec_bytes, s->rec_slab);
     desc_free(p->device, s->desc_entry);
   }
   desc_free(p->device, p->desc_entry);
@@ -599,6 +656,37 @@
   return DVO_AMD_OK;
 }
 
+int dvo_amd_debug_point_records(dvo_amd_pyramid *p, const dvo_amd_mask *mask, float ti, float td, int level, int capacity,
+                                float *rec_a, float *rec_b, float *plain, int *n, int *n_points, int *in_use) {
+  if (!p || level < 0 || level >= p->n_levels || capacity < 0) return DVO_AMD_ERR_INVALID_ARGUMENT;
+  const Selection *sp = nullptr;
+  int rc = pyramid_selection(p, ti, td, mask, &sp);
+  if (rc) return rc;
+  unsigned levels = 0;
+  rc = selection_point_records(p, sp, &levels);
+  if (rc) return rc;
+  const int n_pad = p->lv[level].n_pad;
+  if (n) *n = n_pad;
+  if (n_points) *n_points = sp->n_pts[level];
+  if (in_use) *in_use = (int)(levels >> level & 1u);
+  if (!rec_a && !rec_b && !plain) return DVO_AMD_OK;
+  if (capacity < n_pad) return invalid("dvo_amd_debug_point_records", "capacity " + std::to_string(capacity) + " is below the level's " +
+                                                                          std::to_string(n_pad) + " entries");
+  HIP_TRY(hipSetDevice(p->device));
+  hipStream_t st;
+  rc = device_prep_stream(p->device, &st);
+  if (rc) return rc;
+  const size_t np = (size_t)n_pad;
+  const CompactLevel &c = sp->pts[level];
+  const float *const arrays[6] = {c.z, c.i, c.ix, c.iy, c.tx, c.ty};
+  if (rec_a) HIP_TRY(hipMemcpyAsync(rec_a, sp->rec_a[level], sizeof(float4) * np, hipMemcpyDeviceToHost, st));
+  if (rec_b) HIP_TRY(hipMemcpyAsync(rec_b, sp->rec_b[level], sizeof(float4) * np, hipMemcpyDeviceToHost, st));
+  for (int k = 0; plain && k < 6; ++k)
+    HIP_TRY(hipMemcpyAsync(plain + (size_t)k * np, arrays[k], sizeof(float) * np, hipMemcpyDeviceToHost, st));
+  HIP_TRY(hipStreamSynchronize(st));
+  return DVO_AMD_OK;
+}
+
 int dvo_amd_pyramid_select(dvo_amd_pyramid *p, int level, float ti, float td, int *count, unsigned char *mask) {
   return select_entry(p, level, ti, td, nullptr, count, mask);
 }
diff --git a/dvo_slam_amd/csrc/dvo_tracker.cpp b/dvo_slam_amd/csrc/dvo_tracker.cpp
--- a/dvo_slam_amd/csrc/dvo_tracker.cpp
+++ b/dvo_slam_amd/csrc/dvo_tracker.cpp
@@ -544,6 +544,7 @@
       j.sub_ll = true;
     }
     if (j.have_b) {
+      if (j.rec_levels >> j.level & 1u) w.flags |= kItemPointRecords;
       w.res_blocks = (uint16_t)j.b.n_blocks;
       res_steps = j.b.steps;
       if (j.b.buf) w.flags |= kItemResBuf;
@@ -568,6 +569,7 @@
       res_steps = j.spec_b.steps;
       if (j.spec_b.buf) w.flags |= kItemResBuf;
       w.flags |= kItemUnitWeights;
+      if (j.rec_levels >> nl & 1u) w.flags |= kItemPointRecords;
       make_kt(j.cur->lv[nl], j.spec_b.estimate_after, w.kt);
       f.records = j.slot->records;
       f.n_blocks = w.res_blocks, f.level_blocks = w.res_blocks;
@@ -853,6 +855,7 @@
     rc = pyramid_selection(j.ref, q.ti, q.td, q.mask, &j.sel);
     dvo_amd_mask_release(q.mask);
     if (rc) return rc;
+    if (ctx->point_records && (rc = selection_point_records(j.ref, j.sel, &j.rec_levels)) != DVO_AMD_OK) return rc;
     dvo_amd_result *r = j.result;
     r->n_levels = 0, r->n_iterations = 0, r->n_ticks = 0, r->n_residual_passes = 0, r->alg_bytes = 0.0, r->alg_bytes_discarded = 0.0, r->is_nan = 0;
     if (!r->iterations) r->iterations_capacity = 0;
@@ -1079,6 +1082,7 @@
   ctx->fin_priority = !(fp && fp[0] == '0');
   if (const char *so = getenv("DVO_AMD_SORT_ITEMS")) ctx->sort_items = so[0] != '0';
   if (const char *sp = getenv("DVO_AMD_SHARE_PLACEMENT")) ctx->share_placement = sp[0] == '0' ? 0 : sp[0] == '2' ? 2 : 1;
+  if (const char *pr = getenv("DVO_AMD_POINT_RECORDS")) ctx->point_records = pr[0] != '0';
   const char *sa = getenv("DVO_AMD_SMALL_ARGS");
   ctx->small_args = !(sa && sa[0] == '0');
   const char *hp = getenv("DVO_AMD_HOST_PROF");
diff --git a/dvo_slam_amd/csrc/dvo_types.h b/dvo_slam_amd/csrc/dvo_types.h
--- a/dvo_slam_amd/csrc/dvo_types.h
+++ b/dvo_slam_amd/csrc/dvo_types.h
@@ -61,6 +61,7 @@
   const float *r_zsel;
   const float *r_i, *r_ix, *r_iy;
   const float *tx, *ty;
+  const float4 *rec_a, *rec_b;
 };
 struct CurLevelDesc {
   const float4 *c_a;
@@ -116,6 +117,7 @@
 constexpr unsigned kItemResBuf = 1;
 constexpr unsigned kItemLlBuf = 2;
 constexpr unsigned kItemUnitWeights = 4;
+constexpr unsigned kItemPointRecords = 8;
 static_assert(sizeof(TickItem) == 104, "TickItem is packed to fit many items into one kernel-argument block");
 
 constexpr int kMaxItemsPerLaunch = 62;
@@ -282,6 +284,8 @@
 hipError_t launch_compact(const float *zsel, const float *r_i, const float *r_ix, const float *r_iy, const float *tx, const float *ty, int w,
                           int n, int n_pad, const int2 *block_partials, int *prefix, const int *counters, float *cz, float *ci, float *cix,
                           float *ciy, float *ctx, float *cty, int *cpix, hipStream_t stream);
+hipError_t launch_point_records(const float *cz, const float *ci, const float *cix, const float *ciy, const float *ctx, const float *cty,
+                                int n_pad, float4 *rec_a, float4 *rec_b, int *not_finite, hipStream_t stream);
 hipError_t launch_mask_from_zsel(const float *zsel, int n, int last_dropped, unsigned char *mask, hipStream_t stream);
 hipError_t launch_unpack_plane(const float4 *c_a, const float2 *c_b, int plane, int n, float *dst, hipStream_t stream);
 
diff --git a/include/dvo_amd_debug.h b/include/dvo_amd_debug.h
--- a/include/dvo_amd_debug.h
+++ b/include/dvo_amd_debug.h
@@ -58,6 +58,9 @@
 int dvo_amd_debug_weights_masked(dvo_amd_context *ctx, dvo_amd_pyramid *reference, dvo_amd_pyramid *current, int level,
                                  const float *T, const float *precision_in, const dvo_amd_mask *mask, float *weights,
                                  dvo_amd_q7_probe *tail);
+
+int dvo_amd_debug_point_records(dvo_amd_pyramid *reference, const dvo_amd_mask *mask, float intensity_threshold, float depth_threshold,
+                                int level, int capacity, float *rec_a, float *rec_b, float *plain, int *n, int *n_points, int *in_use);
 
 int dvo_amd_debug_hw_queue(dvo_amd_context *ctx, int *pipe_queue);
 
```

New measurement: 62070. 1.9% lower.
